# andimarafioti/qwen3-tts-cuda-graphs

Hardware: NVIDIA B200
Metric: audio_seconds_per_second (higher is better)
Workload: dtype bf16

## Files before the change

qwen3_tts_cuda_graphs_b200/csrc/fq3_api.cu:

```cuda
#include <cstdio>
#include <cstdlib>
#include <cstring>
#include <string>
#include <array>
#include <vector>

#include "../../include/fq3.h"
#include "fq3_kernel.cuh"

using namespace fq3;

namespace {

thread_local std::string g_err;
int fail(int code, const std::string& msg) {
  g_err = msg;
  return -code;
}
#define CK(call)                                                                                     \
  do {                                                                                               \
    cudaError_t _e = (call);                                                                         \
    if (_e != cudaSuccess)                                                                           \
      return fail(FQ3_E_CUDA, std::string(#call) + ": " + cudaGetErrorString(_e) + " @" + __FILE__ + ":" + \
                                  std::to_string(__LINE__));                                         \
// ... 198 lines not shown
        p.in_buf = BUF_PIN; p.out_buf = BUF_PX; p.w_off = off16(e->desc.s2m_w_off); p.b_off = off16(e->desc.s2m_b_off);
        p.N = e->pr.d.hidden; p.K = e->tk.d.hidden;
        p.plan = plan_id(e, p.N, p.K, false);
        v.push_back(p);
      }
      for (int l = 0; l < L; ++l) push_layer(e, v, e->pr, ST_PRED, l, false, (uint8_t)i, true);
    }
    Phase h{};
    h.type = PH_GEMV; h.stack = ST_PRED; h.aux = (uint8_t)i;
    h.flags = F_PRENORM | F_OUT_F32 | F_L2_KEEP;
    h.in_buf = BUF_PX; h.out_buf = BUF_LOGITS; h.w_off = off16(e->lm_head_offs[i]);
    h.g_off = off16(e->pr.d.final_norm_off); h.N = e->pr.d.vocab; h.K = e->pr.d.hidden;
    h.plan = plan_id(e, h.N, h.K, false);
    v.push_back(h);
    Phase sm{};
    sm.type = PH_SAMPLE; sm.stack = ST_PRED; sm.aux = (uint8_t)i; sm.skind = SMP_PRED;
    v.push_back(sm);
  }
}

void push_talker(std::vector<Phase>& v, fq3_engine* e, bool last_row_head) {
  for (int l = 0; l < e->tk.d.n_layers; ++l) push_layer(e, v, e->tk, ST_TALKER, l, false, 0, false);
  Phase h{};
  h.type = PH_GEMV; h.stack = ST_TALKER;
  h.flags = F_PRENORM | F_OUT_F32 | F_WRITE_NORMED | (last_row_head ? F_LAST_ROW : 0);
  h.in_buf = BUF_TX; h.out_buf = BUF_LOGITS; h.w_off = off16(e->desc.codec_head_off);
  h.g_off = off16(e->tk.d.final_norm_off); h.N = e->tk.d.vocab; h.K = e->tk.d.hidden;
  h.plan = plan_id(e, h.N, h.K, false);
  v.push_back(h);
}

int upload(fq3_engine* e, std::vector<Phase>& v, Phase** d) {
  const uint8_t* arena = reinterpret_cast<const uint8_t*>(e->desc.arena);
  std::vector<std::array<uint32_t, 8>> kinds;
  for (Phase& ph : v) {
    if (ph.type != PH_GEMV) continue;
    const std::array<uint32_t, 8> key{ph.flags, ph.in_buf, ph.out_buf, ph.res_buf, ph.N, ph.K, ph.plan, ph.b_off};
    size_t k = 0;
    while (k < kinds.size() && kinds[k] != key) ++k;
    if (k == kinds.size()) kinds.push_back(key);
    if (k >= (size_t)kMaxKinds) return -1;
    ph.kind = (uint8_t)k;
  }
  for (Phase& ph : v) {
    if (ph.type != PH_GEMV) continue;
    if (ph.N % 8) return -1;
    const uint64_t aoff = (uint64_t)ph.w_off * 16;
    uint64_t ioff = ~0ull;
    for (auto& m : e->tiled_map)
      if (m.first == aoff) ioff = m.second;
    if (ioff == ~0ull) {
      size_t used = 0;
      if (!e->tiled_map.empty()) used = e->tiled_used;
      ioff = used;
      const size_t bytes = (size_t)ph.N * ph.K * 2;
      if (ioff + bytes > e->tiled_bytes) return -1;
      fq3_tile_weights_kernel<<<256, 256>>>(reinterpret_cast<const bf16*>(arena + aoff), reinterpret_cast<uint4*>(e->tiled + ioff), (int)ph.N,
                                            (int)ph.K);
      if (cudaGetLastError() != cudaSuccess) return -1;
      e->tiled_map.push_back({aoff, ioff});
      e->tiled_used = (ioff + bytes + 1023) / 1024 * 1024;
    }
    ph.w_off = off16(ioff);
  }
  if (dalloc(e, d, v.size(), false)) return -1;
  if (cudaMemcpy(*d, v.data(), v.size() * sizeof(Phase), cudaMemcpyHostToDevice) != cudaSuccess) return -1;
  return 0;
}

void fill_common(fq3_engine* e, LaunchParams& p) {
  p.arena = reinterpret_cast<const uint8_t*>(e->desc.arena);
  p.tiled = e->tiled;
  for (int i = 0; i < kNumBufs; ++i) { p.bufs[i] = e->bufs[i]; p.ld[i] = e->ld[i]; }
  p.stacks[0] = e->rt[0];
  p.stacks[1] = e->rt[1];
  p.st = e->d_st;
  p.attn_part = e->attn_part;
  for (size_t i = 0; i < e->plans.size(); ++i) p.plans[i] = e->plans[i];
  p.err = e->err_dev;
  p.n_code_groups = e->desc.n_code_groups;
  p.eos_id = e->desc.eos_id;
  p.has_s2m = e->desc.has_s2m;
  p.max_frames = e->desc.max_frames;
  p.codec_embed = reinterpret_cast<const bf16*>(p.arena + e->desc.codec_embed_off);
  for (int i = 0; i < e->ncb; ++i) p.pred_embeds[i] = reinterpret_cast<const bf16*>(p.arena + e->pred_embed_offs[i]);
  p.pred_logits_all = nullptr;
  p.pos_override = -1;
  p.watchdog_ns = e->watchdog_ns;
  p.debug = (16 << 16) | 32;
  p.prof = e->prof;
  p.prof_cta = e->prof_cta;
  if (const char* d = getenv("FQ3_DEBUG")) p.debug = atoi(d);
  p.n_iters = 1;
  p.stream0 = 0;
  p.wide = 0;
  p.max_streams = e->desc.max_streams;
}

int check_device_fault(fq3_engine* e) {
  if (e->err_host && e->err_host[0] != 0) {
    char b[256];
    snprintf(b, sizeof b, "device watchdog fault: code=%d cta=%d phase=%d detail=%d (1=grid barrier 2=ring full-wait "
                          "3=ring empty-wait 4=frame handshake 5=bad phase)",
             e->err_host[0], e->err_host[1], e->err_host[2], e->err_host[3]);
    return fail(FQ3_E_DEVICE_FAULT, b);
  }
  return 0;
}

int phase_rows_host(const Phase& ph, int n_rows) {
  if (ph.flags & F_LAST_ROW) return 1;
  return (ph.flags & F_ROWS2) ? 2 * n_rows : n_rows;
}

int reserve_epochs(fq3_engine* e, uint64_t span, cudaStream_t s) {
  if (int r = check_device_fault(e)) return r;
  if ((uint64_t)e->epoch + span >= 0xFFFFFF00ull) {
    for (int i = 0; i < kNumBufs; ++i)
      if (e->buf_bytes[i]) fq3_ll_clear_epochs_kernel<<<64, 256, 0, s>>>(reinterpret_cast<LLWord*>(e->bufs[i]), e->buf_bytes[i] / sizeof(LLWord));
    fq3_ll_clear_epochs_kernel<<<64, 256, 0, s>>>(e->attn_part, e->attn_part_bytes / sizeof(LLWord));
    fq3_ctl_clear_epochs_kernel<<<1, 64, 0, s>>>(e->d_st, e->desc.max_streams);
    e->launches += 2;
    CK(cudaGetLastError());
    e->epoch = 1;
  }
  return 0;
}

long carve(fq3_engine* e, LaunchParams& p, const Phase* prog_host) {
  size_t xbytes = 0, gamma_elems = 0;
  for (int i = 0; i < p.n_phases; ++i) {
    const Phase& ph = prog_host[i];
    if (ph.type != PH_GEMV) continue;
    const int M = phase_rows_host(ph, p.n_rows);
    if (M > (p.wide ? kMaxWide : kMaxRows)) return fail(FQ3_E_UNSUPPORTED, "more activation rows than the GEMV stage takes");
    xbytes = std::max(xbytes, (M == 1 && !p.wide) ? (size_t)4 * ph.K : (size_t)M * ((size_t)ph.K * 2 + 64));
    if (ph.flags & F_PRENORM) gamma_elems = std::max(gamma_elems, (size_t)ph.K);
  }
  p.xbuf_bytes = (int)round_up(xbytes, 2048);
  p.prog_bytes = (int)round_up((size_t)kKindBytes + kUnitBytes + (size_t)p.n_phases * sizeof(Phase), 1024);
  p.gam_bytes = (int)round_up(gamma_elems * 2, 1024);
  const long fixed = kHeaderBytes + kScratchBytes + (long)p.xbuf_bytes + (long)p.prog_bytes + (long)kGammaSlots * p.gam_bytes;
  const long budget = e->ring_cap > 0 ? (long)e->smem_max : std::min<long>((long)e->smem_max, 196L * 1024);
  long avail = budget - fixed;
  if (avail < 6L * kStageBytes) avail = (long)e->smem_max - fixed;
  if (e->ring_cap > 0) avail = std::min(avail, e->ring_cap);
  p.n_stages = (int)std::min<long>(kMaxStages, avail / kStageBytes);
  if (p.n_stages < 2) return fail(FQ3_E_INVALID, "not enough shared memory for the weight ring");
  return fixed;
}

int launch(fq3_engine* e, LaunchParams& p, const Phase* prog_host, cudaStream_t s) {
  const int grid = e->G;
  const long fixed = carve(e, p, prog_host);
  if (fixed < 0) return (int)fixed;
  p.n_kinds = 0;
  for (int i = 0; i < p.n_phases; ++i) {
    const Phase& ph = prog_host[i];
    if (ph.type != PH_GEMV) continue;
    if (ph.kind >= kMaxKinds) return fail(FQ3_E_INVALID, "phase kind out of range");
    if (ph.kind >= p.n_kinds) {
      p.n_kinds = ph.kind + 1;
      p.kind_phase[ph.kind] = (uint16_t)i;
    }
  }
  const size_t smem = (size_t)fixed + (size_t)p.n_stages * kStageBytes;
  for (int i = 0; i < p.n_phases; ++i) {
    const Phase& ph = prog_host[i];
    if (ph.type != PH_GEMV) continue;
    Plan& pl = p.plans[ph.plan];
    if (pl.spg > p.n_stages) return fail(FQ3_E_UNSUPPORTED, "K too large for the weight ring");
    const int g_max = pl.g_base + (pl.g_rem ? 1 : 0);
    const bool follow_ref = p.mode == MODE_FRAMES && (p.wide || p.n_rows > 1) && e->ref_stages > 0;
    if (follow_ref && std::min(pl.gpr, g_max) * pl.spg > e->ref_stages) {
      pl.gpr = e->ref_stages / pl.spg;
      pl.wpg = std::max(1, std::min(kConsumerWarps / pl.gpr, pl.nch));
    }
    if (std::min(pl.gpr, g_max) * pl.spg > p.n_stages) {
      pl.gpr = p.n_stages / pl.spg;
      if (!follow_ref) pl.wpg = std::max(1, std::min(kConsumerWarps / pl.gpr, pl.nch));
    }
  }

  const uint64_t span = (uint64_t)p.n_iters * (uint64_t)p.n_phases + 2;
  if ((uint64_t)e->epoch + span >= 0xFFFFFFF0ull) return fail(FQ3_E_INVALID, "LL epochs were not reserved for this launch");
  p.epoch_base = e->epoch;
  e->epoch += (uint32_t)span;
  void* args[] = {&p};
  void* fn = p.wide ? (void*)fq3_stream_kernel<false, true> : (p.prof ? (void*)fq3_stream_kernel<true, false> : (void*)fq3_stream_kernel<false, false>);
  CK(cudaLaunchCooperativeKernel(fn, dim3(grid), dim3(kThreads), args, smem, s));
  e->launches += 1;
  e->frames_rows = (p.mode == MODE_FRAMES && !p.wide) ? p.n_rows : 0;
  return 0;
}

int pack_ll(fq3_engine* e, int buf, int row0, const void* src, int ld_src, int rows, int cols, cudaStream_t s) {
  LLWord* dst = reinterpret_cast<LLWord*>(e->bufs[buf]) + (size_t)row0 * e->ld[buf];
  const int n = rows * cols;
  fq3_pack_ll_kernel<<<std::max(1, std::min(64, (n + 255) / 256)), 256, 0, s>>>(dst, e->ld[buf], reinterpret_cast<const bf16*>(src),
                                                                          ld_src, rows, cols);
  e->launches += 1;
  CK(cudaGetLastError());
  return 0;
}
int unpack_f32(fq3_engine* e, void* dst, int ld_dst, int buf, int row0, int rows, int cols, cudaStream_t s) {
  const LLWord* src = reinterpret_cast<const LLWord*>(e->bufs[buf]) + (size_t)row0 * e->ld[buf];
  const int n = rows * cols;
  fq3_unpack_ll_f32_kernel<<<std::max(1, std::min(64, (n + 255) / 256)), 256, 0, s>>>(reinterpret_cast<float*>(dst), ld_dst, src,
                                                                                e->ld[buf], rows, cols);
  e->launches += 1;
  CK(cudaGetLastError());
  return 0;
}
int unpack_bf16(fq3_engine* e, void* dst, int ld_dst, int buf, int row0, int rows, int cols, cudaStream_t s) {
  const LLWord* src = reinterpret_cast<const LLWord*>(e->bufs[buf]) + (size_t)row0 * e->ld[buf];
  const int n = rows * cols;
  fq3_unpack_ll_bf16_kernel<<<std::max(1, std::min(64, (n + 255) / 256)), 256, 0, s>>>(reinterpret_cast<bf16*>(dst), ld_dst, src,
                                                                                 e->ld[buf], rows, cols);
  e->launches += 1;
  CK(cudaGetLastError());
  return 0;
}

Policy to_policy(const fq3_policy* q) {
  Policy p{};
  p.do_sample = q->do_sample; p.top_k = q->top_k; p.top_p = q->top_p; p.temperature = q->temperature;
  p.rep_pen = q->repetition_penalty; p.min_new_tokens = q->min_new_tokens; p.suppress_tail = q->suppress_tail;
  p.seed = q->seed;
  return p;
}
SubPolicy to_sub(const fq3_subpolicy* q) {
  SubPolicy p{};
  p.do_sample = q->do_sample; p.top_k = q->top_k; p.top_p = q->top_p; p.temperature = q->temperature;
  return p;
}

int sync_pin_layout(fq3_engine* e, int s0, int n, bool to_wpin, cudaStream_t s) {
  const int pb = e->desc.has_s2m ? BUF_PIN : BUF_PX;
  for (int i = s0; i < s0 + n; ++i) {
    if ((e->in_wpin[i] != 0) == to_wpin) continue;
    fq3_wpin_from_pairs_kernel<<<1, 256, 0, s>>>(reinterpret_cast<LLWord*>(e->bufs[BUF_WPIN]), e->ld[BUF_WPIN], reinterpret_cast<LLWord*>(e->bufs[pb]),
                                                 e->ld[pb], i, e->desc.max_streams, to_wpin ? 0 : 1);
    e->launches += 1;
    CK(cudaGetLastError());
    e->in_wpin[i] = to_wpin ? 1 : 0;
  }
  return 0;
}

int check_stack(const fq3_stack_desc& d, const char* name) {
  if (d.head_dim != kHeadDim) return fail(FQ3_E_UNSUPPORTED, std::string(name) + ": head_dim must be 128");
  if (d.hidden % 64 || d.inter % 64) return fail(FQ3_E_UNSUPPORTED, std::string(name) + ": dims must be multiples of 64");
  if (d.n_q_heads % d.n_kv_heads) return fail(FQ3_E_UNSUPPORTED, std::string(name) + ": nq % nkv != 0");
  if (d.n_q_heads / d.n_kv_heads > kGq) return fail(FQ3_E_UNSUPPORTED, std::string(name) + ": more than 2 q heads per kv head");
  if (d.vocab > kMaxVocab) return fail(FQ3_E_UNSUPPORTED, std::string(name) + ": vocab exceeds sampling scratch");
  if (d.vocab % 4) return fail(FQ3_E_UNSUPPORTED, std::string(name) + ": vocab must be a multiple of 4");
  return 0;
}

}

extern "C" {

int fq3_abi_version(void) { return FQ3_ABI_VERSION; }
const char* fq3_last_error(void) { return g_err.c_str(); }

static int create_impl(const fq3_model_desc* desc, fq3_engine* e);

int fq3_create(const fq3_model_desc* desc, fq3_engine** out) {
  if (!desc || !out) return fail(FQ3_E_INVALID, "null argument");
  *out = nullptr;
  fq3_engine* e = new fq3_engine();
  const int r = create_impl(desc, e);
  if (r) {
    const std::string msg = g_err;
    fq3_destroy(e);
    g_err = msg;
    return r;
  }
  *out = e;
  return 0;
}

static int create_impl(const fq3_model_desc* desc, fq3_engine* e) {
  if (desc->abi_version != FQ3_ABI_VERSION) return fail(FQ3_E_INVALID, "ABI version mismatch");
  if (int r = check_stack(desc->talker, "talker")) return r;
  if (int r = check_stack(desc->predictor, "predictor")) return r;
  if (desc->n_code_groups < 2 || desc->n_code_groups > FQ3_MAX_CODE_GROUPS) return fail(FQ3_E_INVALID, "n_code_groups");
  if (desc->max_streams < 1) return fail(FQ3_E_INVALID, "max_streams");
  if (!desc->has_s2m && desc->talker.hidden != desc->predictor.hidden)
    return fail(FQ3_E_INVALID, "talker/predictor widths differ but no small_to_mtp projection given");
  e->desc = *desc;
  CK(cudaGetDevice(&e->dev));
  int sms = 0, smem_optin = 0, coop = 0;
  CK(cudaDeviceGetAttribute(&sms, cudaDevAttrMultiProcessorCount, e->dev));
  CK(cudaDeviceGetAttribute(&smem_optin, cudaDevAttrMaxSharedMemoryPerBlockOptin, e->dev));
  CK(cudaDeviceGetAttribute(&coop, cudaDevAttrCooperativeLaunch, e->dev));
  if (!coop) return fail(FQ3_E_UNSUPPORTED, "device lacks cooperative launch");
  e->n_sms = sms;
  e->G = std::min(sms, 128);
  if (const char* g = getenv("FQ3_GRID")) e->G = std::max(1, std::min(sms, atoi(g)));
  if (const char* rk = getenv("FQ3_RING_KB")) e->ring_cap = std::max(16L, atol(rk)) * 1024L;
  if (const char* pc = getenv("FQ3_PROF")) {
    e->prof_cta = atoi(pc);
    if (dalloc(e, &e->prof, 512 * 160 * 2)) return -FQ3_E_CUDA;
  }
  if (const char* w = getenv("FQ3_WATCHDOG_MS")) e->watchdog_ns = (unsigned long long)atoll(w) * 1000000ull;
  e->smem_max = (size_t)smem_optin;
  CK(cudaFuncSetAttribute(fq3_stream_kernel<false, false>, cudaFuncAttributeMaxDynamicSharedMemorySize, smem_optin));
  CK(cudaFuncSetAttribute(fq3_stream_kernel<true, false>, cudaFuncAttributeMaxDynamicSharedMemorySize, smem_optin));
  CK(cudaFuncSetAttribute(fq3_stream_kernel<false, true>, cudaFuncAttributeMaxDynamicSharedMemorySize, smem_optin));
  int occ = 0;
  CK(cudaOccupancyMaxActiveBlocksPerMultiprocessor(&occ, fq3_stream_kernel<false, false>, kThreads, smem_optin));
  if (occ < 1) return fail(FQ3_E_UNSUPPORTED, "stream kernel does not fit on an SM");

  e->ncb = desc->n_code_groups - 1;
  e->tk.d = desc->talker;
  e->pr.d = desc->predictor;
  e->tk.offs.assign(desc->talker.layer_offs, desc->talker.layer_offs + (size_t)desc->talker.n_layers * 8);
  e->pr.offs.assign(desc->predictor.layer_offs, desc->predictor.layer_offs + (size_t)desc->predictor.n_layers * 8);
  e->lm_head_offs.assign(desc->lm_head_offs, desc->lm_head_offs + e->ncb);
  e->pred_embed_offs.assign(desc->pred_embed_offs, desc->pred_embed_offs + e->ncb);
  e->tk.d.layer_offs = nullptr;
  e->pr.d.layer_offs = nullptr;

  const int B = desc->max_streams;
  const int R = std::max(2 * B, 2 * kMaxRows);
  e->max_rows = R;
  const uint8_t* arena = reinterpret_cast<const uint8_t*>(desc->arena);
  for (int s = 0; s < 2; ++s) {
    const StackHost& sh = s == 0 ? e->tk : e->pr;
    StackRt& r = e->rt[s];
    r.hidden = sh.d.hidden; r.inter = sh.d.inter; r.n_layers = sh.d.n_layers; r.nq = sh.d.n_q_heads;
    r.nkv = sh.d.n_kv_heads; r.vocab = sh.d.vocab; r.eps = sh.d.rms_eps; r.max_pos = sh.d.max_pos;
    r.rope_len = sh.d.rope_len; r.n_slots = B;
    const size_t n = (size_t)sh.d.n_layers * B * sh.d.n_kv_heads * sh.d.max_pos * kHeadDim;
    if (dalloc(e, &r.kcache, n)) return -FQ3_E_CUDA;
    if (dalloc(e, &r.vcache, n)) return -FQ3_E_CUDA;
    r.rope_cos = reinterpret_cast<const bf16*>(arena + sh.d.rope_cos_off);
    r.rope_sin = reinterpret_cast<const bf16*>(arena + sh.d.rope_sin_off);
  }
  auto mk = [&](int id, int width, size_t elt, int rows) -> int {
    void* q = nullptr;
    if (dalloc(e, reinterpret_cast<uint8_t**>(&q), (size_t)rows * width * elt)) return -1;
    e->bufs[id] = q;
    e->ld[id] = width;
    e->buf_bytes[id] = (size_t)rows * width * elt;
    return 0;
  };
  const int Ht = e->tk.d.hidden, Hp = e->pr.d.hidden;
  const size_t LL = sizeof(LLWord);
  if (mk(BUF_TX, Ht / 2, LL, R) || mk(BUF_TQKV, e->tk.qkvdim() / 2, LL, R) || mk(BUF_TATT, e->tk.qdim() / 2, LL, R) ||
      mk(BUF_TACT, e->tk.d.inter / 2, LL, R) || mk(BUF_PX, Hp / 2, LL, R) || mk(BUF_PQKV, e->pr.qkvdim() / 2, LL, R) ||
      mk(BUF_PATT, e->pr.qdim() / 2, LL, R) || mk(BUF_PACT, e->pr.d.inter / 2, LL, R) ||
      mk(BUF_LOGITS, std::max(e->tk.d.vocab, e->pr.d.vocab) / 2, LL, R) || mk(BUF_HID, Ht, 2, R))
    return -FQ3_E_CUDA;
  e->buf_bytes[BUF_HID] = 0;
  if (desc->has_s2m) {
    if (mk(BUF_PIN, Ht / 2, LL, R)) return -FQ3_E_CUDA;
  } else {
    e->bufs[BUF_PIN] = e->bufs[BUF_PX];
    e->ld[BUF_PIN] = e->ld[BUF_PX];
  }
  if (mk(BUF_WPIN, Ht / 2, LL, 2 * B)) return -FQ3_E_CUDA;
  e->lin_words = 32768;
  if (mk(BUF_LIN_IN, e->lin_words, LL, kMaxRows) || mk(BUF_LIN_OUT, e->lin_words, LL, kMaxRows) ||
      mk(BUF_LIN_RES, e->lin_words, LL, kMaxRows))
    return -FQ3_E_CUDA;
  const int nqmax = std::max(e->tk.d.n_q_heads, e->pr.d.n_q_heads);
  e->attn_part_bytes = (size_t)R * nqmax * kMaxSplits * kPartStride * sizeof(LLWord);
  if (dalloc(e, &e->attn_part, (size_t)R * nqmax * kMaxSplits * kPartStride)) return -FQ3_E_CUDA;
  if (dalloc(e, &e->pred_logits_all, (size_t)e->ncb * e->pr.d.vocab)) return -FQ3_E_CUDA;
  if (dalloc(e, &e->seen_scratch, (size_t)kMaxVocab * 4)) return -FQ3_E_CUDA;
  CK(cudaHostAlloc(reinterpret_cast<void**>(&e->err_host), 64, cudaHostAllocMapped));
  memset(e->err_host, 0, 64);
  CK(cudaHostGetDevicePointer(reinterpret_cast<void**>(&e->err_dev), e->err_host, 0));
  e->h_st.resize(B);
  e->in_wpin.assign(B, 0);
  e->spol_on.assign(B, 0);
  e->text_rows.assign(B, 0);
  e->text_open.assign(B, 0);
  if (dalloc(e, &e->d_st, B)) return -FQ3_E_CUDA;
  if (dalloc(e, &e->d_spol, B)) return -FQ3_E_CUDA;
  for (int b = 0; b < B; ++b) {
    StreamState& s = e->h_st[b];
    memset(&s, 0, sizeof s);
    bf16 *tr = nullptr, *pe = nullptr;
    if (dalloc(e, &tr, (size_t)e->tk.d.max_pos * Ht)) return -FQ3_E_CUDA;
    if (dalloc(e, &pe, (size_t)Ht)) return -FQ3_E_CUDA;
    if (dalloc(e, &s.held, (size_t)Ht)) return -FQ3_E_CUDA;
    if (dalloc(e, &s.codes, (size_t)desc->max_frames * desc->n_code_groups)) return -FQ3_E_CUDA;
    if (dalloc(e, &s.seen, (size_t)round_up(e->tk.d.vocab, 16))) return -FQ3_E_CUDA;
    s.trailing = tr;
    s.pad_embed = pe;
  }
  CK(cudaMemcpy(e->d_st, e->h_st.data(), sizeof(StreamState) * B, cudaMemcpyHostToDevice));
  auto gemv_bytes = [&](const StackHost& sh) {
    return (size_t)sh.d.n_layers * ((size_t)sh.qkvdim() * sh.d.hidden + (size_t)sh.d.hidden * sh.qdim() + 3ull * sh.d.hidden * sh.d.inter) * 2;
  };
  e->tiled_bytes = gemv_bytes(e->tk) + gemv_bytes(e->pr) + (size_t)e->tk.d.vocab * e->tk.d.hidden * 2 +
                   (size_t)e->ncb * e->pr.d.vocab * e->pr.d.hidden * 2 + (desc->has_s2m ? (size_t)e->pr.d.hidden * e->tk.d.hidden * 2 : 0) +
                   1024 * (size_t)(8 * (e->tk.d.n_layers + e->pr.d.n_layers) + e->ncb + 8);
  if (dalloc(e, &e->tiled, e->tiled_bytes, false)) return -FQ3_E_CUDA;
  std::vector<Phase>& v = e->h_frames;
  push_predictor(v, e, false);
  push_talker(v, e, false);
  {
    Phase s{};
    s.type = PH_SAMPLE; s.stack = ST_TALKER; s.skind = SMP_TALKER;
    v.push_back(s);
  }
  push_predictor(e->h_pred, e, true);
  push_talker(e->h_talker, e, false);
  push_talker(e->h_prefill, e, true);
  {
    Phase s{};
    s.type = PH_SAMPLE; s.stack = ST_TALKER; s.skind = SMP_PREFILL;
    e->h_prefill.push_back(s);
  }
  push_predictor_wide(e->h_wide, e);
  push_talker(e->h_wide, e, false);
  {
    Phase s{};
    s.type = PH_SAMPLE; s.stack = ST_TALKER; s.skind = SMP_TALKER;
    e->h_wide.push_back(s);
  }
  if (g_plan_fail) { g_plan_fail = false; return fail(FQ3_E_UNSUPPORTED, "a GEMV shape of this model cannot be partitioned (odd N or K % 64)"); }
  e->n_frames_ph = (int)e->h_frames.size();
  e->n_pred_ph = (int)e->h_pred.size();
  e->n_talker_ph = (int)e->h_talker.size();
  e->n_prefill_ph = (int)e->h_prefill.size();
  e->n_wide_ph = (int)e->h_wide.size();
  if (upload(e, e->h_wide, &e->d_wide)) return fail(FQ3_E_CUDA, "wide program upload");
  {
    const int kmax = std::max(e->tk.kmax(), e->pr.kmax());
    const long fixed = kHeaderBytes + kScratchBytes + (long)round_up((size_t)kKindBytes + kUnitBytes + (size_t)e->n_wide_ph * sizeof(Phase), 1024) +
                       (long)kGammaSlots * (long)round_up((size_t)std::max(e->tk.d.hidden, e->pr.d.hidden) * 2, 1024);
    const long spg_max = ((long)kmax * 16 + kStageBytes - 1) / kStageBytes;
    const long avail = (long)e->smem_max - fixed - std::max(4L, spg_max + 1) * kStageBytes - 2048;
    e->wide_rows = (int)std::max<long>(0, std::min<long>(avail / ((long)kmax * 2 + 64), kMaxWide));
  }
  {
    LaunchParams q{};
    q.n_phases = e->n_frames_ph; q.n_rows = 1;
    if (carve(e, q, e->h_frames.data()) < 0) return -FQ3_E_INVALID;
    e->ref_stages = q.n_stages;
  }
  if (upload(e, e->h_frames, &e->d_frames) || upload(e, e->h_pred, &e->d_pred) || upload(e, e->h_talker, &e->d_talker) ||
      upload(e, e->h_prefill, &e->d_prefill))
    return fail(FQ3_E_CUDA, "program upload / weight tiling (matrix rows must be a multiple of 8)");
  if (dalloc(e, &e->d_linear, 1)) return -FQ3_E_CUDA;
  CK(cudaDeviceSynchronize());
  return 0;
}

int fq3_destroy(fq3_engine* e) {
  if (!e) return 0;
  cudaDeviceSynchronize();
// ... 313 lines not shown
  if (V <= 0 || V > kMaxVocab) return fail(FQ3_E_UNSUPPORTED, "vocab exceeds sampling scratch");
  SampleArgs a{};
  a.V = V; a.do_sample = policy->do_sample; a.top_k = policy->top_k; a.top_p = policy->top_p;
  a.temperature = policy->temperature; a.rep_pen = policy->repetition_penalty; a.seen = nullptr;
  a.suppress_start = policy->suppress_tail > 0 ? std::max(0, V - policy->suppress_tail) : V;
  a.eos = eos_id; a.suppress_eos = suppress_eos; a.round_bf16 = flags & 1; a.seed = policy->seed; a.draw = draw_index;
  a.next_emb = nullptr; a.emb_row_bytes = 0;
  fq3_sample_kernel<<<1, kConsumerThreads, 0, (cudaStream_t)stream>>>(
      reinterpret_cast<const float*>(logits_f32), a, reinterpret_cast<const long long*>(history_i64), n_history,
      e->seen_scratch, reinterpret_cast<long long*>(out_token_i64));
  e->launches += 1;
  CK(cudaGetLastError());
  return 0;
}

int fq3_apply_repetition_penalty(fq3_engine* e, void* logits_f32, int V, const void* history_i64, int n_history,
                                 float penalty, int flags, void* stream) {
  if (!e || !logits_f32) return fail(FQ3_E_INVALID, "bad arguments");
  if (V <= 0 || V > kMaxVocab * 4) return fail(FQ3_E_UNSUPPORTED, "vocab exceeds scratch");
  if (penalty == 1.0f || n_history <= 0 || !history_i64) return 0;
  fq3_rep_penalty_kernel<<<1, kConsumerThreads, 0, (cudaStream_t)stream>>>(
      reinterpret_cast<float*>(logits_f32), V, reinterpret_cast<const long long*>(history_i64), n_history, penalty,
      flags & 1, e->seen_scratch);
  e->launches += 1;
  CK(cudaGetLastError());
  return 0;
}

int fq3_decode_frames(fq3_engine* e, int n_streams, int n_frames, const fq3_policy* policy, const fq3_subpolicy* sub,
                      void* stream) {
  if (!e || !policy || !sub) return fail(FQ3_E_INVALID, "bad decode arguments");
  if (n_streams < 1 || n_streams > e->desc.max_streams) return fail(FQ3_E_INVALID, "n_streams out of range");
  if (n_frames <= 0) return 0;
  int wide_from = 3;
  if (const char* wf = getenv("FQ3_WIDE_FROM")) wide_from = std::max(1, atoi(wf));
  if ((n_streams >= wide_from && e->wide_rows > kMaxRows / 2) || 2 * n_streams > kMaxRows) {
    if (e->wide_rows <= kMaxRows / 2)
      return fail(FQ3_E_UNSUPPORTED, "more than four lock-step streams do not fit this model's staging buffer: decode in groups of fq3_lockstep_group()");
    const int n_groups = (n_streams + e->wide_rows - 1) / e->wide_rows;
    const int per = (n_streams + n_groups - 1) / n_groups;
    if (int r = sync_pin_layout(e, 0, n_streams, true, (cudaStream_t)stream)) return r;
    for (int s0 = 0; s0 < n_streams; s0 += per) {
      const int n = std::min(per, n_streams - s0);
      if (int r = reserve_epochs(e, (uint64_t)n_frames * (uint64_t)e->n_wide_ph + 2, (cudaStream_t)stream)) return r;
      LaunchParams p{};
      fill_common(e, p);
      p.prog = e->d_wide;
      p.n_phases = e->n_wide_ph;
      p.mode = MODE_FRAMES;
      p.wide = 1;
      p.n_rows = n;
      p.stream0 = s0;
      p.n_iters = n_frames;
      p.pol = to_policy(policy);
      p.spol = spol_for(e, s0, n);
      p.sub = to_sub(sub);
      if (int r = launch(e, p, e->h_wide.data(), (cudaStream_t)stream)) return r;
    }
    return 0;
  }
  if (int r = reserve_epochs(e, (uint64_t)n_frames * (uint64_t)e->n_frames_ph + 2, (cudaStream_t)stream)) return r;
  if (int r = sync_pin_layout(e, 0, n_streams, false, (cudaStream_t)stream)) return r;
  LaunchParams p{};
  fill_common(e, p);
  p.prog = e->d_frames;
  p.n_phases = e->n_frames_ph;
  p.mode = MODE_FRAMES;
  p.n_rows = n_streams;
  p.n_iters = n_frames;
  p.pol = to_policy(policy);
  p.spol = spol_for(e, 0, n_streams);
  p.sub = to_sub(sub);
  return launch(e, p, e->h_frames.data(), (cudaStream_t)stream);
}

int fq3_set_decode_grid(fq3_engine* e, int n_ctas) {
  if (!e) return fail(FQ3_E_INVALID, "null engine");
  if (n_ctas <= 0 || n_ctas == e->G || n_ctas == e->n_sms) return 0;
  return fail(FQ3_E_UNSUPPORTED, "the decode grid is fixed at engine creation (FQ3_GRID)");
}
int fq3_assemble_prompt(fq3_engine* e, const void* tp_rows, const void* desc_i32x4, int n_rows, const void* spk_rows,
                        const void* ref_codes_i32, void* out_bf16, void* stream) {
  if (!e || !desc_i32x4 || !out_bf16 || n_rows < 0) return fail(FQ3_E_INVALID, "bad assemble_prompt arguments");
  if (n_rows == 0) return 0;
  PromptTables tb{};
  const uint8_t* arena = reinterpret_cast<const uint8_t*>(e->desc.arena);
  tb.codec_embed = reinterpret_cast<const bf16*>(arena + e->desc.codec_embed_off);
  for (int i = 0; i < e->ncb; ++i) tb.pred_embeds[i] = reinterpret_cast<const bf16*>(arena + e->pred_embed_offs[i]);
  tb.ncb = e->ncb;
  fq3_assemble_prompt_kernel<<<n_rows, 256, 0, (cudaStream_t)stream>>>(
      reinterpret_cast<const bf16*>(tp_rows), reinterpret_cast<const int4*>(desc_i32x4), e->tk.d.hidden, tb,
      reinterpret_cast<const bf16*>(spk_rows), reinterpret_cast<const int*>(ref_codes_i32), e->desc.n_code_groups,
      reinterpret_cast<bf16*>(out_bf16));
  e->launches += 1;
  CK(cudaGetLastError());
  return 0;
}

int fq3_lockstep_group(const fq3_engine* e) { return e ? std::max(e->wide_rows, kMaxRows / 2) : 0; }
int fq3_reduced_grid(const fq3_engine* e) { return (e && e->G < e->n_sms) ? e->G : 0; }

int fq3_clear_fault(fq3_engine* e, void* stream) {
  if (!e) return fail(FQ3_E_INVALID, "null engine");
  cudaStreamSynchronize((cudaStream_t)stream);
  if (cudaGetLastError() != cudaSuccess) return fail(FQ3_E_CUDA, "the CUDA context is in an error state: rebuild the engine");
  if (e->err_host) memset(e->err_host, 0, 64);
  for (int i = 0; i < kNumBufs; ++i)
    if (e->buf_bytes[i]) CK(cudaMemsetAsync(e->bufs[i], 0, e->buf_bytes[i], (cudaStream_t)stream));
  CK(cudaMemsetAsync(e->attn_part, 0, e->attn_part_bytes, (cudaStream_t)stream));
  e->epoch = 1;
  return 0;
}

int fq3_debug_set_epoch(fq3_engine* e, uint32_t epoch) {
  if (!e || epoch == 0) return fail(FQ3_E_INVALID, "bad arguments");
  e->epoch = epoch;
  return 0;
}

int fq3_debug_read_talker_logits(fq3_engine* e, int idx, void* out_f32, void* stream) {
  if (int r = check_stream(e, idx)) return r;
  if (!out_f32) return fail(FQ3_E_INVALID, "null output");
  if (idx >= e->frames_rows)
    return fail(FQ3_E_INVALID, "the last launch was not a reference-shaped fq3_decode_frames launch that ran this stream");
  return unpack_f32(e, out_f32, e->tk.d.vocab, BUF_LOGITS, idx, 1, e->tk.d.vocab, (cudaStream_t)stream);
}

int fq3_get_status(fq3_engine* e, int idx, fq3_status* out, void* stream) {
  if (int r = check_stream(e, idx)) return r;
  cudaError_t se = cudaStreamSynchronize((cudaStream_t)stream);
  if (int r = check_device_fault(e)) return r;
  if (se != cudaSuccess) return fail(FQ3_E_CUDA, std::string("stream sync: ") + cudaGetErrorString(se));
  StreamState s;
  CK(cudaMemcpy(&s, e->d_st + idx, sizeof s, cudaMemcpyDeviceToHost));
  out->n_frames = s.n_frames; out->done = s.done; out->position = s.position; out->gen_step = s.gen_step;
  out->token = s.token; out->error = e->err_host[0];
  return 0;
}

int fq3_read_codes(fq3_engine* e, int idx, int first, int n, int32_t* codes_out, void* stream) {
  if (int r = check_stream(e, idx)) return r;
  if (first < 0 || n < 0 || first + n > e->desc.max_frames) return fail(FQ3_E_INVALID, "frame range");
  if (n == 0) return 0;
  const int g = e->desc.n_code_groups;
  CK(cudaMemcpyAsync(codes_out, e->h_st[idx].codes + (size_t)first * g, (size_t)n * g * 4, cudaMemcpyDeviceToHost,
                     (cudaStream_t)stream));
  CK(cudaStreamSynchronize((cudaStream_t)stream));
  return 0;
}

int fq3_debug_read_prof(fq3_engine* e, long long* out, int n_words) {
  if (!e || !e->prof) return fail(FQ3_E_INVALID, "profiling not enabled (FQ3_PROF)");
  CK(cudaDeviceSynchronize());
  CK(cudaMemcpy(out, e->prof, sizeof(long long) * std::min(n_words, 512 * 160 * 2), cudaMemcpyDeviceToHost));
  CK(cudaMemset(e->prof, 0, sizeof(long long) * 512 * 160 * 2));
  return 0;
}

int fq3_last_hidden(fq3_engine* e, int row, void* out_bf16, void* stream) {
  if (!e || !out_bf16 || row < 0 || row >= e->max_rows) return fail(FQ3_E_INVALID, "bad arguments");
  const int Ht = e->tk.d.hidden;
  CK(cudaMemcpyAsync(out_bf16, reinterpret_cast<const bf16*>(e->bufs[BUF_HID]) + (size_t)row * e->ld[BUF_HID], (size_t)Ht * 2,
                     cudaMemcpyDeviceToDevice, (cudaStream_t)stream));
  return 0;
}

void* fq3_codes_device_ptr(fq3_engine* e, int idx) {
  if (!e || idx < 0 || idx >= e->desc.max_streams) return nullptr;
  return e->h_st[idx].codes;
}

int fq3_linear(fq3_engine* e, const void* W, const void* x, void* y, int M, int N, int K, int flags, const void* gamma,
               float eps, const void* bias, const void* residual, void* stream) {
  if (!e || !W || !x || !y) return fail(FQ3_E_INVALID, "null argument");
  if (M < 1 || M > kMaxRows) return fail(FQ3_E_UNSUPPORTED, "M must be in [1, 8]");
  if (K % 64 || N < 2 || (N & 1) || K / 2 > e->lin_words || N / 2 > e->lin_words)
    return fail(FQ3_E_UNSUPPORTED, "K must be a multiple of 64 and N even");
  if ((flags & 8) && (N % 4)) return fail(FQ3_E_INVALID, "SwiGLU needs N to be a multiple of 4");
  Plan lin_plan{};
  if (!make_plan(e->G, N, K, (flags & 8) != 0, &lin_plan)) return fail(FQ3_E_UNSUPPORTED, "shape cannot be partitioned");
  cudaStream_t s = (cudaStream_t)stream;
  if (int r = reserve_epochs(e, 3, s)) return r;
  const size_t img_bytes = (size_t)((N + 7) / 8 * 8) * K * 2;
  if (img_bytes > e->lin_img_bytes) {
    CK(cudaStreamSynchronize(s));
    if (e->lin_img) {
      cudaFree(e->lin_img);
      for (void*& q : e->owned) if (q == e->lin_img) q = nullptr;
      e->lin_img = nullptr;
    }
    e->lin_img_bytes = 0;
    if (dalloc(e, &e->lin_img, img_bytes, false)) return -FQ3_E_CUDA;
    e->lin_img_bytes = img_bytes;
  }
  fq3_tile_weights_kernel<<<256, 256, 0, s>>>(reinterpret_cast<const bf16*>(W), reinterpret_cast<uint4*>(e->lin_img), N, K);
  e->launches += 1;
  CK(cudaGetLastError());
  Phase ph{};
  ph.type = PH_GEMV;
  ph.flags = F_ABSPTR | ((flags & 1) ? F_PRENORM : 0) | ((flags & 2) ? F_BIAS : 0) | ((flags & 4) ? F_RESID : 0) |
             ((flags & 8) ? F_SWIGLU : 0) | ((flags & 16) ? F_OUT_F32 : 0) | ((flags & 32) ? F_SILU : 0);
  ph.in_buf = BUF_LIN_IN; ph.out_buf = BUF_LIN_OUT; ph.res_buf = BUF_LIN_RES;
  ph.N = (uint32_t)N; ph.K = (uint32_t)K;
  ph.plan = (uint8_t)(kMaxPlans - 1);
  CK(cudaMemcpyAsync(e->d_linear, &ph, sizeof ph, cudaMemcpyHostToDevice, s));
  LaunchParams p{};
  fill_common(e, p);
  p.prog = e->d_linear;
  p.n_phases = 1;
  p.mode = MODE_LINEAR;
  p.n_rows = M;
  const int No = (flags & 8) ? N / 2 : N;
  if (int r = pack_ll(e, BUF_LIN_IN, 0, x, K, M, K, s)) return r;
  if (flags & 4) {
    if (!residual) return fail(FQ3_E_INVALID, "residual flag without a residual pointer");
    if (int r = pack_ll(e, BUF_LIN_RES, 0, residual, No, M, No, s)) return r;
  }
  p.lin_W = e->lin_img; p.lin_gamma = gamma; p.lin_bias = bias; p.lin_eps = eps;
  p.plans[kMaxPlans - 1] = lin_plan;
  if (int r = launch(e, p, &ph, s)) return r;
  if (flags & 16) return unpack_f32(e, y, No, BUF_LIN_OUT, 0, M, No, s);
  return unpack_bf16(e, y, No, BUF_LIN_OUT, 0, M, No, s);
}

}
```

qwen3_tts_cuda_graphs_b200/csrc/fq3_common.cuh:

```cuda
#pragma once
#include <cuda_bf16.h>
#include <cuda_runtime.h>
#include <stdint.h>

namespace fq3 {

typedef __nv_bfloat16 bf16;

constexpr int kConsumerWarps = 12;
constexpr int kConsumerThreads = kConsumerWarps * 32;
constexpr int kThreads = kConsumerThreads + 128;
constexpr int kProducerRegs = 56;
constexpr int kConsumerRegs = 152;
constexpr int kPollWarps = 8;
constexpr int kPollThreads = kPollWarps * 32;
constexpr int kMaxStages = 16;
constexpr int kGroupRows = 8;
constexpr int kChunkK = 32;
constexpr int kBlockBytes = kGroupRows * kChunkK * 2;
constexpr int kStageBytes = 16 * 1024;
constexpr int kStageChunks = kStageBytes / kBlockBytes;
constexpr int kHeadDim = 128;
constexpr int kMaxRows = 8;
constexpr int kMaxWide = 16;
constexpr int kMaxSplits = 16;
constexpr int kSplitLen = 4 * kConsumerWarps;
constexpr int kPartStride = 132;
constexpr int kNumBufs = 16;
constexpr int kMaxVocab = 5120;
constexpr int kScratchBytes = 24 * 1024;
constexpr int kEmptyOffset = 128;
constexpr int kCtlOffset = 256;
constexpr int kFramePosIdx = 8;
constexpr int kFrameDoneIdx = 8 + kMaxWide;
constexpr int kRedOffset = 512;
constexpr int kGFullOffset = 1024;
constexpr int kGEmptyOffset = 1056;
constexpr int kStreamConstOffset = 1088;
constexpr int kHeaderBytes = 2048;
constexpr int kGammaSlots = 4;
constexpr int kMaxPlans = 24;

typedef uint2 LLWord;

enum PhaseType : uint8_t { PH_END = 0, PH_GEMV = 1, PH_ATTN = 2, PH_SAMPLE = 3 };
enum StackId : uint8_t { ST_TALKER = 0, ST_PRED = 1 };
enum SampleKind : uint8_t { SMP_PRED = 0, SMP_TALKER = 1, SMP_PREFILL = 2, SMP_PRED_ONLY = 3 };

enum PhaseFlags : uint16_t {
  F_PRENORM = 1,
  F_BIAS = 2,
  F_RESID = 4,
  F_SWIGLU = 8,
  F_OUT_F32 = 16,
  F_ROWS2 = 32,
  F_LAST_ROW = 64,
  F_WRITE_NORMED = 128,
  F_L2_KEEP = 256,
  F_ABSPTR = 512,
  F_SILU = 1024,
  F_PASS0A = 2048,
  F_WPIN_B = 4096,
  F_IN_PREV = 8192
};

struct __align__(16) Phase {
  uint8_t type;
  uint8_t stack;
  uint8_t layer;
  uint8_t aux;
  uint16_t flags;
  uint8_t in_buf, out_buf;
  uint32_t w_off;
  uint32_t g_off;
  uint32_t b_off;
  uint32_t N;
  uint32_t K;
  uint8_t res_buf;
  uint8_t skind;
  uint8_t plan;
  uint8_t kind;
};
static_assert(sizeof(Phase) == 32, "Phase must stay 32 bytes");

enum BufId : uint8_t {
  BUF_TX = 0, BUF_TQKV, BUF_TATT, BUF_TACT, BUF_PX, BUF_PQKV, BUF_PATT, BUF_PACT, BUF_PIN,
  BUF_LOGITS, BUF_HID, BUF_LIN_IN, BUF_LIN_OUT, BUF_LIN_RES, BUF_WPIN, BUF_COUNT
};

struct Plan {
  int g_base, g_rem;
  int wpg;
  int gpr;
  int spg;
  int nch;
  int ro_shift;
  float inv_k;
};
constexpr int kMaxKinds = 32;
struct __align__(16) KindDesc {
  const LLWord* in;
  int Kq, flags;
  LLWord* out;
  const LLWord* res;
  const uint32_t* bias;
  int ldout, ldres;
  int g, grp0, wpg, gpr;
  int spg, nch, ro_shift, n_stages;
  float eps, inv_k;
  int n_rounds, wpgrp;
  int M, n_words, K, fast;
  int ldin, norm, pad0, pad1;
};
static_assert(sizeof(KindDesc) == 128, "KindDesc is eight 16-byte lines");
struct __align__(16) UnitDesc {
  int wgrp, kp;
  int ch0, ch1;
};
constexpr int kKindBytes = kMaxKinds * (int)sizeof(KindDesc);
constexpr int kUnitBytes = kMaxKinds * kConsumerWarps * (int)sizeof(UnitDesc);

struct StackRt {
  int hidden, inter, n_layers, nq, nkv, vocab;
  float eps;
  int max_pos;
  int rope_len;
  int n_slots;
  bf16* kcache;
  bf16* vcache;
  const bf16* rope_cos;
  const bf16* rope_sin;
};

struct StreamState {
  int token;
  int position;
  int gen_step;
  int n_frames;
  int done;
  int n_pad;
  int rope_delta;
  int n_trailing;
  int text_open;
  unsigned long long draws;
  const bf16* trailing;
  const bf16* pad_embed;
  bf16* held;
  int* codes;
  uint8_t* seen;
  int cur_codes[32];
  LLWord ctl[4];
};

struct Policy {
  int do_sample, top_k;
  float top_p, temperature, rep_pen;
  int min_new_tokens, suppress_tail;
  unsigned long long seed;
};
struct SubPolicy {
  int do_sample, top_k;
  float top_p, temperature;
};
struct StreamPolicy {
  int on;
  Policy pol;
};

enum Mode : int { MODE_FRAMES = 0, MODE_TALKER_STEP = 1, MODE_PREDICTOR = 2, MODE_PREFILL = 3, MODE_LINEAR = 4 };

struct LaunchParams {
  const Phase* prog;
  int n_phases;
  int n_kinds;
  uint16_t kind_phase[kMaxKinds];
  int n_iters;
  int mode;
  int n_rows;
  int wide;
  int max_streams;
  int stream0;
  int pos_override;
  int pf_pos0, pf_n_pad, pf_rope_delta, pf_final;
  const uint8_t* arena;
  const uint8_t* tiled;
  void* bufs[kNumBufs];
  int ld[kNumBufs];
  StackRt stacks[2];
  StreamState* st;
  Policy pol;
  SubPolicy sub;
  const StreamPolicy* spol;
  LLWord* attn_part;
  int* err;
// ... 21 lines not shown
```

qwen3_tts_cuda_graphs_b200/csrc/fq3_kernel.cuh:

```cuda
#pragma once
#include "fq3_common.cuh"

namespace fq3 {

__device__ __forceinline__ uint32_t smem_u32(const void* p) { return (uint32_t)__cvta_generic_to_shared(p); }

__device__ __forceinline__ void mbar_init(uint64_t* bar, uint32_t count) {
  asm volatile("mbarrier.init.shared::cta.b64 [%0], %1;" ::"r"(smem_u32(bar)), "r"(count) : "memory");
}
__device__ __forceinline__ void mbar_arrive(uint64_t* bar) {
  asm volatile("mbarrier.arrive.shared::cta.b64 _, [%0];" ::"r"(smem_u32(bar)) : "memory");
}
__device__ __forceinline__ void mbar_arrive_expect_tx(uint64_t* bar, uint32_t bytes) {
  asm volatile("mbarrier.arrive.expect_tx.shared::cta.b64 _, [%0], %1;" ::"r"(smem_u32(bar)), "r"(bytes) : "memory");
}
__device__ __forceinline__ bool mbar_try_wait(uint64_t* bar, uint32_t parity) {
  uint32_t ok;
  asm volatile(
      "{\n\t.reg .pred p;\n\t"
      "mbarrier.try_wait.parity.shared::cta.b64 p, [%1], %2;\n\t"
      "selp.u32 %0, 1, 0, p;\n\t}"
      : "=r"(ok)
      : "r"(smem_u32(bar)), "r"(parity)
      : "memory");
// ... 28 lines not shown
  asm volatile("createpolicy.fractional.L2::evict_last.b64 %0, 1.0;" : "=l"(p));
  return p;
}

__device__ __forceinline__ void cbar_sync() { asm volatile("bar.sync 1, %0;" ::"n"(kConsumerThreads) : "memory"); }

__device__ __forceinline__ unsigned long long globaltimer_ns() {
  unsigned long long t;
  asm volatile("mov.u64 %0, %%globaltimer;" : "=l"(t));
  return t;
}
__device__ __forceinline__ int ld_volatile_shared_i32(const int* p) {
  int v;
  asm volatile("ld.volatile.shared.s32 %0, [%1];" : "=r"(v) : "r"(smem_u32(p)) : "memory");
  return v;
}
__device__ __forceinline__ void st_volatile_shared_i32(int* p, int v) {
  asm volatile("st.volatile.shared.s32 [%0], %1;" ::"r"(smem_u32(p)), "r"(v) : "memory");
}
__device__ __forceinline__ uint4 lds128(uint32_t addr) {
  uint4 v;
  asm volatile("ld.shared.v4.u32 {%0, %1, %2, %3}, [%4];" : "=r"(v.x), "=r"(v.y), "=r"(v.z), "=r"(v.w) : "r"(addr));
  return v;
}

__device__ __forceinline__ LLWord ll_ld(const LLWord* p) {
  LLWord w;
  asm volatile("ld.relaxed.gpu.global.v2.u32 {%0, %1}, [%2];" : "=r"(w.x), "=r"(w.y) : "l"(p) : "memory");
  return w;
}
__device__ __forceinline__ void ll_ld2(const LLWord* p, LLWord& a, LLWord& b) {
  asm volatile("ld.relaxed.gpu.global.v4.u32 {%0, %1, %2, %3}, [%4];" : "=r"(a.x), "=r"(a.y), "=r"(b.x), "=r"(b.y) : "l"(p) : "memory");
}
__device__ __forceinline__ void ll_st(LLWord* p, uint32_t payload, uint32_t ep) {
  const unsigned long long val = ((unsigned long long)ep << 32) | payload;
  asm volatile("red.relaxed.gpu.global.max.u64 [%0], %1;" ::"l"(p), "l"(val) : "memory");
}
__device__ __forceinline__ void ll_st2(LLWord* p, uint32_t pay0, uint32_t pay1, uint32_t ep) {
  ll_st(p, pay0, ep);
  ll_st(p + 1, pay1, ep);
}
__device__ __forceinline__ void ll_stf(LLWord* p, float v, uint32_t ep) { ll_st(p, __float_as_uint(v), ep); }

__device__ __forceinline__ float bf16r(float x) { return __bfloat162float(__float2bfloat16_rn(x)); }
__device__ __forceinline__ float bf_lo(uint32_t w) { return __uint_as_float(w << 16); }
__device__ __forceinline__ float bf_hi(uint32_t w) { return __uint_as_float(w & 0xffff0000u); }
__device__ __forceinline__ uint32_t pack_bf16x2(float lo, float hi) {
  __nv_bfloat162 v = __floats2bfloat162_rn(lo, hi);
  return *reinterpret_cast<uint32_t*>(&v);
}
__device__ __forceinline__ float warp_sum(float v) {
#pragma unroll
  for (int o = 16; o > 0; o >>= 1) v += __shfl_xor_sync(0xffffffffu, v, o);
  return v;
}
__device__ __forceinline__ float warp_max(float v) {
#pragma unroll
  for (int o = 16; o > 0; o >>= 1) v = fmaxf(v, __shfl_xor_sync(0xffffffffu, v, o));
  return v;
}
struct Smem {
  uint64_t* full;
  uint64_t* empty;
  int* ctl;
  float* red;
  unsigned char* scratch;
  KindDesc* kinds;
  UnitDesc* units;
  Phase* prog;
  unsigned char* gam;
  unsigned char* xbuf;
  unsigned char* ring;
};

__device__ __forceinline__ Smem carve_smem(unsigned char* base, const LaunchParams& p) {
  Smem s;
  s.full = reinterpret_cast<uint64_t*>(base);
  s.empty = reinterpret_cast<uint64_t*>(base + kEmptyOffset);
  s.ctl = reinterpret_cast<int*>(base + kCtlOffset);
  s.red = reinterpret_cast<float*>(base + kRedOffset);
  s.scratch = base + kHeaderBytes;
  s.kinds = reinterpret_cast<KindDesc*>(s.scratch + kScratchBytes);
  s.units = reinterpret_cast<UnitDesc*>(s.scratch + kScratchBytes + kKindBytes);
  s.prog = reinterpret_cast<Phase*>(s.scratch + kScratchBytes + kKindBytes + kUnitBytes);
  s.gam = s.scratch + kScratchBytes + p.prog_bytes;
  s.xbuf = s.gam + kGammaSlots * p.gam_bytes;
  s.ring = s.xbuf + p.xbuf_bytes;
  return s;
}

__device__ __noinline__ void device_fault(const LaunchParams& p, int code, int phase, int detail) {
  volatile int* e = p.err;
  if (e[0] == 0) {
    e[1] = blockIdx.x;
    e[2] = phase;
    e[3] = detail;
    e[0] = code;
  }
  __threadfence_system();
  asm volatile("trap;");
}

struct Spin {
  unsigned long long t0;
  unsigned n;
  __device__ __forceinline__ Spin() : t0(0), n(0) {}
  __device__ __forceinline__ void tick(const LaunchParams& p, int code, int phase, int detail) {
    if ((++n & 0x3ff) == 0) {
      unsigned long long t = globaltimer_ns();
      if (t0 == 0) t0 = t;
      else if (t - t0 > p.watchdog_ns) device_fault(p, code, phase, detail);
    }
  }
};

__device__ __noinline__ void mbar_wait_slow(uint64_t* bar, uint32_t parity, const LaunchParams& p, int code, int phase) {
  Spin s;
  while (!mbar_try_wait(bar, parity)) s.tick(p, code, phase, (int)parity);
}
__device__ __forceinline__ void mbar_wait(uint64_t* bar, uint32_t parity, const LaunchParams& p, int code, int phase) {
  if (mbar_try_wait(bar, parity)) return;
  mbar_wait_slow(bar, parity, p, code, phase);
}

__device__ __noinline__ LLWord ll_spin(const LLWord* ptr, uint32_t ep, const LaunchParams& p, int phase) {
  Spin s;
  LLWord w;
  unsigned tries = 0;
  do {
    if (++tries > 4) __nanosleep(40);
    s.tick(p, DE_LL_WAIT, phase, (int)ep);
    w = ll_ld(ptr);
  } while (w.y != ep);
  return w;
}
__device__ __forceinline__ uint32_t ll_check(LLWord w, const LLWord* ptr, uint32_t ep, const LaunchParams& p, int phase) {
  if (ep != 0 && w.y != ep) w = ll_spin(ptr, ep, p, phase);
  return w.x;
}
__device__ __forceinline__ uint32_t ll_wait(const LLWord* ptr, uint32_t ep, const LaunchParams& p, int phase) {
  return ll_check(ll_ld(ptr), ptr, ep, p, phase);
}

#ifndef FQ3_CHECKS
#define FQ3_CHECKS 0
#endif
#if FQ3_CHECKS
#define FQ3_ASSERT(cond, pidx, detail) do { if (!(cond)) device_fault(p, DE_ASSERT, (pidx), (detail)); } while (0)
#else
#define FQ3_ASSERT(cond, pidx, detail) do { } while (0)
#endif

__device__ __forceinline__ void prof_cta_time(const LaunchParams& p, int pidx, int k) {
  if (p.prof && p.prof_cta == -2 && threadIdx.x == 0 && pidx >= 0 && pidx < 512)
    p.prof[((size_t)pidx * 160 + blockIdx.x) * 2 + k] = (long long)globaltimer_ns();
}
__device__ __forceinline__ void prof_warp_time(const LaunchParams& p, int pidx, int k) {
  if (p.prof && p.prof_cta == -3 && blockIdx.x == 0 && (threadIdx.x & 31) == 0 && pidx >= 0 && pidx < 512)
    p.prof[((size_t)pidx * 160 + 16 * (k >> 1) + (threadIdx.x >> 5)) * 2 + (k & 1)] = clock64();
}
__device__ __forceinline__ void prof_mark(const LaunchParams& p, int pidx, int slot, int thread = 0) {
  if (p.prof && (int)threadIdx.x == thread && (int)blockIdx.x == p.prof_cta && pidx >= 0 && pidx < 512) p.prof[(size_t)pidx * 16 + slot] = clock64();
}
#ifndef FQ3_WIDE_PROF
#define FQ3_WIDE_PROF 0
#endif
__device__ __forceinline__ void prof_acc(const LaunchParams& p, int cat, long long& t, int thread = 0) {
  if (FQ3_WIDE_PROF && p.prof && (int)threadIdx.x == thread && (int)blockIdx.x == p.prof_cta) {
    const long long now = clock64();
    p.prof[cat] += now - t;
    t = now;
  }
}
constexpr int kProfLeader = (kConsumerWarps - 1) * 32;

__device__ __forceinline__ float silu_f(float x) { return __fdividef(x, 1.f + __expf(-x)); }

__device__ __forceinline__ int phase_rows(const Phase& ph, const LaunchParams& p) {
  return (ph.flags & F_ROWS2) ? 2 * p.n_rows : p.n_rows;
}

__device__ __forceinline__ uint2 ldg_keep_u2(const void* ptr, uint64_t pol) {
  uint2 v;
  asm volatile("ld.global.nc.L2::cache_hint.v2.u32 {%0, %1}, [%2], %3;" : "=r"(v.x), "=r"(v.y) : "l"(ptr), "l"(pol));
  return v;
}

__device__ __forceinline__ Phase load_phase(const Phase* prog_smem, int i) {
  union { Phase ph; uint4 q[2]; } u;
  const uint32_t a = smem_u32(prog_smem + i);
  u.q[0] = lds128(a);
  u.q[1] = lds128(a + 16u);
  return u.ph;
}

struct Ctx {
  uint32_t full, empty, red, scratch, xs, ring, gfull, gempty, gam;
  int n_stages, gam_bytes;
  uint32_t kinds, units, xhalf;
  const Phase* prog;
};
__device__ __forceinline__ Ctx make_ctx(unsigned char* smem_base, const LaunchParams& p) {
  const Smem sm = carve_smem(smem_base, p);
  Ctx c;
  c.full = smem_u32(sm.full);
  c.empty = smem_u32(sm.empty);
  c.red = smem_u32(sm.red);
  c.scratch = smem_u32(sm.scratch);
  c.xs = smem_u32(sm.xbuf);
  c.ring = smem_u32(sm.ring);
  c.n_stages = p.n_stages;
  c.gfull = smem_u32(smem_base + kGFullOffset);
  c.gempty = smem_u32(smem_base + kGEmptyOffset);
  c.gam = smem_u32(sm.gam);
  c.gam_bytes = p.gam_bytes;
  c.xhalf = (uint32_t)p.xbuf_bytes / 2u;
  c.kinds = smem_u32(sm.kinds);
  c.units = smem_u32(sm.units);
  c.prog = sm.prog;
  return c;
}
__device__ __forceinline__ bool mbar_try_wait_a(uint32_t bar, uint32_t parity) {
  uint32_t ok;
  asm volatile(
      "{\n\t.reg .pred p;\n\t"
      "mbarrier.try_wait.parity.shared::cta.b64 p, [%1], %2;\n\t"
      "selp.u32 %0, 1, 0, p;\n\t}"
      : "=r"(ok)
      : "r"(bar), "r"(parity)
      : "memory");
  return ok != 0;
}
__device__ __forceinline__ void mbar_arrive_a(uint32_t bar) { asm volatile("mbarrier.arrive.shared::cta.b64 _, [%0];" ::"r"(bar) : "memory"); }
__device__ __forceinline__ float lds_f32(uint32_t a) {
  float v;
  asm volatile("ld.shared.f32 %0, [%1];" : "=f"(v) : "r"(a));
  return v;
}
__device__ __forceinline__ float2 lds_f32x2(uint32_t a) {
  float2 v;
  asm volatile("ld.shared.v2.f32 {%0, %1}, [%2];" : "=f"(v.x), "=f"(v.y) : "r"(a));
  return v;
}
__device__ __forceinline__ float4 lds_f32x4(uint32_t a) {
  float4 v;
  asm volatile("ld.shared.v4.f32 {%0, %1, %2, %3}, [%4];" : "=f"(v.x), "=f"(v.y), "=f"(v.z), "=f"(v.w) : "r"(a));
  return v;
}
__device__ __forceinline__ void sts_f32(uint32_t a, float v) { asm volatile("st.shared.f32 [%0], %1;" ::"r"(a), "f"(v) : "memory"); }
__device__ __forceinline__ void sts_f32x2(uint32_t a, float v0, float v1) { asm volatile("st.shared.v2.f32 [%0], {%1, %2};" ::"r"(a), "f"(v0), "f"(v1) : "memory"); }
__device__ __forceinline__ void sts_u32(uint32_t a, uint32_t v) { asm volatile("st.shared.u32 [%0], %1;" ::"r"(a), "r"(v) : "memory"); }
__device__ __forceinline__ uint32_t lds_u32(uint32_t a) {
  uint32_t v;
  asm volatile("ld.shared.u32 %0, [%1];" : "=r"(v) : "r"(a));
  return v;
}
__device__ __forceinline__ uint2 lds_u32x2(uint32_t a) {
  uint2 v;
  asm volatile("ld.shared.v2.u32 {%0, %1}, [%2];" : "=r"(v.x), "=r"(v.y) : "r"(a));
  return v;
}
__device__ __forceinline__ void group_bar_sync(int id, int nthreads) { asm volatile("bar.sync %0, %1;" ::"r"(id), "r"(nthreads) : "memory"); }

__device__ __forceinline__ void mma_bf16(float (&c)[4], uint32_t a0, uint32_t a1, uint32_t a2, uint32_t a3, uint32_t b0, uint32_t b1) {
  asm volatile(
      "mma.sync.aligned.m16n8k16.row.col.f32.bf16.bf16.f32 {%0, %1, %2, %3}, {%4, %5, %6, %7}, {%8, %9}, {%0, %1, %2, %3};"
      : "+f"(c[0]), "+f"(c[1]), "+f"(c[2]), "+f"(c[3])
      : "r"(a0), "r"(a1), "r"(a2), "r"(a3), "r"(b0), "r"(b1));
}

struct RingCur {
  int slot;
  uint32_t lap;
  __device__ __forceinline__ void advance(int n, int n_stages) {
    slot += n;
    while (slot >= n_stages) { slot -= n_stages; lap ^= 1u; }
  }
};

__device__ __forceinline__ int small_div(int a, int b) { return (int)__fdividef((float)a + 0.5f, (float)b); }

struct Slab {
  int g, grp0;
  int n_stages;
};
__device__ __forceinline__ Slab get_slab(const Phase& ph, const LaunchParams& p) {
  const Plan& pl = p.plans[ph.plan];
  const int cta = blockIdx.x;
  Slab s;
  s.g = pl.g_base + (cta < pl.g_rem ? 1 : 0);
  s.grp0 = cta * pl.g_base + min(cta, pl.g_rem);
  s.n_stages = s.g * pl.spg;
  return s;
}

__device__ __forceinline__ void resolve_kind(const LaunchParams& p, const Phase& ph, KindDesc& kd) {
  const Plan& pl = p.plans[ph.plan];
  const Slab sb = get_slab(ph, p);
  const uint32_t flags = ph.flags;
  int M = (flags & F_ROWS2) ? 2 * p.n_rows : p.n_rows, row_off = 0;
  if (flags & F_LAST_ROW) { row_off = M - 1; M = 1; }
  const int K = (int)ph.K;
  const int wpin_row = p.stream0 + ((flags & F_WPIN_B) ? p.max_streams : 0);
  if (ph.in_buf == BUF_WPIN) row_off += wpin_row;
  kd.ldin = p.ld[ph.in_buf];
  kd.in = reinterpret_cast<const LLWord*>(p.bufs[ph.in_buf]) + (size_t)row_off * kd.ldin;
  kd.Kq = K >> 2;
  kd.flags = (int)flags;
  kd.out = reinterpret_cast<LLWord*>(p.bufs[ph.out_buf]);
  kd.ldout = p.ld[ph.out_buf];
  kd.ldres = (flags & F_RESID) ? p.ld[ph.res_buf] : 0;
  kd.res = (flags & F_RESID) ? reinterpret_cast<const LLWord*>(p.bufs[ph.res_buf]) + (size_t)(ph.res_buf == BUF_WPIN ? wpin_row : 0) * kd.ldres : nullptr;
  kd.bias = nullptr;
  if (flags & F_BIAS)
    kd.bias = reinterpret_cast<const uint32_t*>((flags & F_ABSPTR) ? p.lin_bias : static_cast<const void*>(p.arena + (size_t)ph.b_off * 16));
// ... 609 lines not shown
        if (g8 + 8 < M) res_pre[1] = ll_ld(kd.res + (size_t)(g8 + 8) * kd.ldres + f_word).x;
      }
      if (flags & F_BIAS) bias_pre = __ldg(kd.bias + f_word);
    }
  }
  {
    long long* tpp = (FQ3_WIDE_PROF && p.prof) ? &tp : nullptr;
    if (K <= 1024) load_x_rows_impl<6, 1, true>(p, flags, kd.in, kd.ldin, gsrc, kd.eps, K, M, ep_in, pidx, c.xs, c.red, tpp);
    else if (K <= 2048) load_x_rows_impl<3, 2, true>(p, flags, kd.in, kd.ldin, gsrc, kd.eps, K, M, ep_in, pidx, c.xs, c.red, tpp);
    else load_x_rows_impl<2, 3, true>(p, flags, kd.in, kd.ldin, gsrc, kd.eps, K, M, ep_in, pidx, c.xs, c.red, tpp);
  }
  if (norm && lane == 0) mbar_arrive_a(gemptyb);

  const int wgrp = ud.wgrp, kp = ud.kp, ch0 = ud.ch0, ch1 = ud.ch1;
  const int wpg = kd.wpg, gpr = kd.gpr, spg = kd.spg, wpgrp = kd.wpgrp;
  const bool w_act = wgrp < gpr;
  const uint32_t rstride = xrow_stride(K);
  const uint32_t xlo = c.xs + (uint32_t)min(g8, M - 1) * rstride + (uint32_t)t * 16u;
  const uint32_t xhi = c.xs + (uint32_t)min(g8 + 8, M - 1) * rstride + (uint32_t)t * 16u;
  const uint32_t lane_w = (uint32_t)lane * 16u;
  const uint32_t pdst = c.scratch + (uint32_t)((wgrp * wpg + kp) * 64 + lane) * 8u;
#pragma unroll 1
  for (int r = 0; r < kd.n_rounds; ++r) {
    if (r != 0) cbar_sync();
    const int gi = r * gpr + wgrp;
    if (!(w_act && gi < kd.g)) continue;
    RingCur my = cur;
    my.advance(gi * spg + (ch0 >> 5), c.n_stages);
    {
      const uint32_t fb = c.full + (uint32_t)my.slot * 8u;
      Spin spin;
      while (!mbar_try_wait_a(fb, my.lap)) spin.tick(p, DE_FULL_WAIT, pidx, my.slot);
    }
    uint32_t wa = c.ring + lane_w + (uint32_t)my.slot * kStageBytes + (uint32_t)(ch0 & (kStageChunks - 1)) * kBlockBytes;
    float acc[4] = {0.f, 0.f, 0.f, 0.f}, acc2[4] = {0.f, 0.f, 0.f, 0.f};
    int ch = ch0;
    long long tq = (FQ3_WIDE_PROF && p.prof) ? clock64() : 0ll;
    if (FQ3_WIDE_PROF && p.prof) { tq = tp; prof_acc(p, 8, tq, kProfLeader); }
#pragma unroll 1
    while (ch < ch1) {
      if (ch != ch0 && (ch & (kStageChunks - 1)) == 0) {
        my.advance(1, c.n_stages);
        const uint32_t fb = c.full + (uint32_t)my.slot * 8u;
        Spin spin;
        while (!mbar_try_wait_a(fb, my.lap)) spin.tick(p, DE_FULL_WAIT, pidx, my.slot);
        wa = c.ring + lane_w + (uint32_t)my.slot * kStageBytes;
      }
      const int ce = min(ch1, (ch | (kStageChunks - 1)) + 1);
      uint32_t xa = (uint32_t)ch * kXBlock;
      uint4 wv = lds128(wa), xl = lds128(xlo + xa), xh = lds128(xhi + xa);
#pragma unroll 2
      for (int n = ce - ch - 1; n > 0; --n) {
        wa += kBlockBytes;
        xa += kXBlock;
        const uint4 wn = lds128(wa), xln = lds128(xlo + xa), xhn = lds128(xhi + xa);
        mma_bf16(acc, xl.x, xh.x, xl.y, xh.y, wv.x, wv.y);
        mma_bf16(acc2, xl.z, xh.z, xl.w, xh.w, wv.z, wv.w);
        wv = wn; xl = xln; xh = xhn;
      }
      mma_bf16(acc, xl.x, xh.x, xl.y, xh.y, wv.x, wv.y);
      mma_bf16(acc2, xl.z, xh.z, xl.w, xh.w, wv.z, wv.w);
      wa += kBlockBytes;
      ch = ce;
    }
    float y[4] = {acc[0] + acc2[0], acc[1] + acc2[1], acc[2] + acc2[2], acc[3] + acc2[3]};
    prof_acc(p, 9, tq, kProfLeader);
    if (wpg > 1) {
      if (kp != 0) {
        sts_f32x2(pdst, y[0], y[1]);
        sts_f32x2(pdst + 256u, y[2], y[3]);
      }
      group_bar_sync(2 + wgrp, wpg * 32);
      if (kp == 1) {
        if (lane == 0) {
          int rs = cur.slot + gi * spg;
          while (rs >= c.n_stages) rs -= c.n_stages;
          for (int s2 = 0; s2 < spg; ++s2) {
            mbar_arrive_a(c.empty + (uint32_t)rs * 8u);
            if (++rs == c.n_stages) rs = 0;
          }
        }
      } else if (kp == 0) {
        if (wpg <= 4) {
#pragma unroll
          for (int k2 = 1; k2 < 4; ++k2) {
            if (k2 < wpg) {
              const float2 v0 = lds_f32x2(pdst + (uint32_t)k2 * 512u), v1 = lds_f32x2(pdst + (uint32_t)k2 * 512u + 256u);
              y[0] += v0.x; y[1] += v0.y; y[2] += v1.x; y[3] += v1.y;
            }
          }
        } else {
          const float2 v0 = tree_parts(y[0], y[1], pdst, 512u, wpg), v1 = tree_parts(y[2], y[3], pdst + 256u, 512u, wpg);
          y[0] = v0.x; y[1] = v0.y; y[2] = v1.x; y[3] = v1.y;
        }
      }
    }
    prof_acc(p, 10, tq, kProfLeader);
    if (kp == 0) {
      const int f_word = (kd.grp0 + gi) * wpgrp + f_sub;
#pragma unroll
      for (int h = 0; h < 2; ++h) {
        const int row = g8 + 8 * h;
        const bool f_lane = row < M && t_ok && f_word < n_words;
        const float y0 = y[2 * h], y1 = y[2 * h + 1];
        uint32_t res0 = res_pre[h], bias0 = bias_pre;
        if (f_lane && r != 0) {
          if (flags & F_RESID) res0 = ll_ld(kd.res + (size_t)row * kd.ldres + f_word).x;
          if (flags & F_BIAS) bias0 = __ldg(kd.bias + f_word);
        }
        float lo, hi;
        if (flags & F_SWIGLU) {
          const float e = bf16r(bf16r(silu_f(bf16r(y0))) * bf16r(y1));
          lo = e;
          hi = __shfl_down_sync(0xffffffffu, e, 1);
        } else {
          lo = y0; hi = y1;
          if (flags & F_BIAS) { lo += bf_lo(bias0); hi += bf_hi(bias0); }
          lo = bf16r(lo); hi = bf16r(hi);
          if (flags & F_SILU) { lo = bf16r(silu_f(lo)); hi = bf16r(silu_f(hi)); }
        }
        if (flags & F_RESID) { lo = bf16r(bf_lo(res0) + lo); hi = bf16r(bf_hi(res0) + hi); }
        if (f_lane) ll_st(kd.out + (size_t)row * kd.ldout + f_word, pack_bf16x2(lo, hi), ep);
      }
      prof_acc(p, 11, tq, kProfLeader);
      if (wpg == 1) {
        __syncwarp();
        if (lane == 0) {
          int rs = cur.slot + gi * spg;
          while (rs >= c.n_stages) rs -= c.n_stages;
          for (int s2 = 0; s2 < spg; ++s2) {
            mbar_arrive_a(c.empty + (uint32_t)rs * 8u);
            if (++rs == c.n_stages) rs = 0;
          }
        }
      }
    }
  }
  cur.advance(kd.n_stages, c.n_stages);
  gst = ((gst & 1u) ^ 1u) | 2u;
  prof_acc(p, 3, tp);
  if (FQ3_WIDE_PROF && p.prof && tid == 0 && (int)blockIdx.x == p.prof_cta) p.prof[6] += 1;
}

template <bool PROF>
__device__ __forceinline__ bool gemv_phase_produce(const Ctx& c, const Phase& ph, const LaunchParams& p, int* ctl, RingCur& cur, RingCur& gcur, uint32_t& issued,
                                                   uint32_t& gissued, int pidx, uint64_t pol_stream, uint64_t pol_keep, uint64_t pol_gamma) {
  const Slab sb = get_slab(ph, p);
  if (sb.g == 0) return true;
  const int K = (int)ph.K;
  const uint32_t gbytes = (uint32_t)K * 16u;
  const unsigned char* W = ((ph.flags & F_ABSPTR) ? reinterpret_cast<const unsigned char*>(p.lin_W) : p.tiled + (size_t)ph.w_off * 16) +
                           (size_t)sb.grp0 * gbytes;
  const uint64_t pol = (ph.flags & F_L2_KEEP) ? pol_keep : pol_stream;
  if (PROF && (int)blockIdx.x == p.prof_cta && pidx < 512) p.prof[(size_t)pidx * 16 + 4] = clock64();
  if (ph.flags & F_PRENORM) {
    const unsigned char* gp = (ph.flags & F_ABSPTR) ? reinterpret_cast<const unsigned char*>(p.lin_gamma) : p.arena + (size_t)ph.g_off * 16;
    const uint32_t gfullb = c.gfull + (uint32_t)gcur.slot * 8u, gemptyb = c.gempty + (uint32_t)gcur.slot * 8u;
    Spin spin;
    while (!mbar_try_wait_a(gemptyb, gcur.lap ^ 1u)) {
      if (ld_volatile_shared_i32(ctl) < 0) return false;
      __nanosleep(100);
      spin.tick(p, DE_EMPTY_WAIT, pidx, 100 + gcur.slot);
    }
    if (ld_volatile_shared_i32(ctl) < 0) return false;
    asm volatile("mbarrier.arrive.expect_tx.shared::cta.b64 _, [%0], %1;" ::"r"(gfullb), "r"((uint32_t)K * 2u) : "memory");
    bulk_g2s_a(c.gam + (uint32_t)gcur.slot * (uint32_t)c.gam_bytes, gp, (uint32_t)K * 2u, gfullb, pol_gamma);
    gcur.advance(1, kGammaSlots);
    ++gissued;
  }
#pragma unroll 1
  for (int gi = 0; gi < sb.g; ++gi) {
#pragma unroll 1
    for (uint32_t off = 0; off < gbytes; off += kStageBytes) {
      const uint32_t bytes = min((uint32_t)kStageBytes, gbytes - off);
      const uint32_t fullb = c.full + (uint32_t)cur.slot * 8u, emptyb = c.empty + (uint32_t)cur.slot * 8u;
      Spin spin;
      while (!mbar_try_wait_a(emptyb, cur.lap ^ 1u)) {
        if (ld_volatile_shared_i32(ctl) < 0) return false;
        __nanosleep(100);
        spin.tick(p, DE_EMPTY_WAIT, pidx, cur.slot);
      }
      if (ld_volatile_shared_i32(ctl) < 0) return false;
      asm volatile("mbarrier.arrive.expect_tx.shared::cta.b64 _, [%0], %1;" ::"r"(fullb), "r"(bytes) : "memory");
      bulk_g2s_a(c.ring + (uint32_t)cur.slot * kStageBytes, W + (size_t)gi * gbytes + off, bytes, fullb, pol);
      cur.advance(1, c.n_stages);
      ++issued;
    }
  }
  if (PROF && (int)blockIdx.x == p.prof_cta && pidx < 512) p.prof[(size_t)pidx * 16 + 5] = clock64();
  return true;
}

struct Group {
  int first_row, nrows, slot, pos0, n_pad, rope_delta;
};
__device__ __forceinline__ int num_groups(const LaunchParams& p) { return p.mode == MODE_PREFILL ? 1 : p.n_rows; }
__device__ __forceinline__ Group get_group(const Phase& ph, const LaunchParams& p, int g, const int* frame_pos) {
  Group r;
  if (p.mode == MODE_PREFILL) {
    r.first_row = 0; r.nrows = p.n_rows; r.slot = p.stream0; r.pos0 = p.pf_pos0; r.n_pad = p.pf_n_pad;
    r.rope_delta = p.pf_rope_delta;
    return r;
  }
  r.nrows = (ph.flags & F_ROWS2) ? 2 : 1;
  r.first_row = g * r.nrows;
  r.slot = p.stream0 + g;
  if (ph.stack == ST_TALKER) {
    r.pos0 = min((p.pos_override >= 0) ? p.pos_override : frame_pos[g], p.stacks[ST_TALKER].max_pos - 1);
    const int* sconst = frame_pos + (kStreamConstOffset - kCtlOffset) / 4 - kFramePosIdx;
    r.n_pad = sconst[g];
    r.rope_delta = sconst[kMaxWide + g];
  } else {
    r.pos0 = (ph.flags & (F_ROWS2 | F_PASS0A)) ? 0 : (int)ph.aux + 1;
    r.n_pad = 0;
    r.rope_delta = 0;
  }
  return r;
}
__device__ __forceinline__ int num_splits(int L, int cap) {
  const int want = (L + kSplitLen - 1) / kSplitLen;
  return max(1, min(want, cap));
}

struct RopeRegs {
  uint2 g2, c2, s2;
};
__device__ __forceinline__ RopeRegs rope_load(const bf16* gamma, const bf16* cosp, const bf16* sinp, int lane) {
  RopeRegs r;
  const uint64_t keep = policy_evict_last();
  r.g2 = ldg_keep_u2(gamma + lane * 4, keep);
  r.c2 = ldg_keep_u2(cosp + lane * 4, keep);
  r.s2 = ldg_keep_u2(sinp + lane * 4, keep);
  return r;
}
__device__ __forceinline__ void head_norm_rope(float (&x)[4], const RopeRegs& rr, float eps, int lane) {
  const uint2 g2 = rr.g2, c2 = rr.c2, s2 = rr.s2;
  float ss = x[0] * x[0] + x[1] * x[1] + x[2] * x[2] + x[3] * x[3];
  ss = warp_sum(ss);
  const float rs = rsqrtf(ss * (1.f / kHeadDim) + eps);
  const float g[4] = {bf_lo(g2.x), bf_hi(g2.x), bf_lo(g2.y), bf_hi(g2.y)};
  const float c[4] = {bf_lo(c2.x), bf_hi(c2.x), bf_lo(c2.y), bf_hi(c2.y)};
  const float sn[4] = {bf_lo(s2.x), bf_hi(s2.x), bf_lo(s2.y), bf_hi(s2.y)};
  float y[4];
#pragma unroll
  for (int i = 0; i < 4; ++i) y[i] = bf16r(bf16r(x[i] * rs) * g[i]);
#pragma unroll
  for (int i = 0; i < 4; ++i) {
    const float partner = __shfl_xor_sync(0xffffffffu, y[i], 16);
    const float rot = (lane < 16) ? -partner : partner;
    x[i] = bf16r(bf16r(y[i] * c[i]) + bf16r(rot * sn[i]));
  }
}

__device__ __forceinline__ void ll_head_wait(const LLWord* src, uint32_t ep, LLWord& a, LLWord& b, const LaunchParams& p, int phase) {
  ll_ld2(src, a, b);
  if (ep == 0) return;
  Spin spin;
  unsigned tries = 0;
  while (__any_sync(0xffffffffu, a.y != ep || b.y != ep)) {
    if (++tries > 4) __nanosleep(40);
    spin.tick(p, DE_LL_WAIT, phase, (int)ep);
    ll_ld2(src, a, b);
  }
}

constexpr int kGq = 2;
constexpr int kAttnPre = 2;
constexpr int kAttnShort = 2 * kAttnPre * kConsumerWarps;

template <bool PROF>
__device__ __forceinline__ void attn_row(const Phase& ph, const LaunchParams& p, unsigned char* smem_base, const Group& gr, int r, int kvh, int sp,
                                      int nsplit, uint32_t ep, int pidx) {
  const Smem sm = carve_smem(smem_base, p);
  const StackRt& S = p.stacks[ph.stack];
  const int warp = threadIdx.x >> 5, lane = threadIdx.x & 31;
  const int gq = S.nq / S.nkv;
  const int qb = ph.stack == ST_TALKER ? BUF_TQKV : BUF_PQKV, ab = ph.stack == ST_TALKER ? BUF_TATT : BUF_PATT;
  const LLWord* qkv = reinterpret_cast<const LLWord*>(p.bufs[qb]) + (size_t)gr.first_row * p.ld[qb];
  const int ldq = p.ld[qb];
  constexpr int HW = kHeadDim / 2;
  const size_t head_base = (((size_t)ph.layer * S.n_slots + gr.slot) * S.nkv + kvh) * (size_t)S.max_pos * kHeadDim;
  bf16* Kc = S.kcache + head_base;
  bf16* Vc = S.vcache + head_base;
  const int pos = gr.pos0 + r;
  FQ3_ASSERT(pos >= 0 && pos < S.max_pos && gr.n_pad >= 0 && gq <= kGq, pidx, 200000 + pos);
  const int L = pos + 1 - gr.n_pad;
  FQ3_ASSERT(r >= 0 && r < kMaxRows && sp >= 0 && sp < nsplit && nsplit <= kMaxSplits, pidx, 210000 + sp);
  const int per = (L + nsplit - 1) / nsplit;
  const int a = gr.n_pad + sp * per;
  const int b = min(a + per, pos + 1);
  float* qs = reinterpret_cast<float*>(sm.scratch);
  uint4* fresh = reinterpret_cast<uint4*>(sm.scratch + 1024);
  float* wp = reinterpret_cast<float*>(sm.scratch + 1024 + 4096);
  const uint32_t ep_in = ep - 1;
  const int hw = lane >> 4, dl = lane & 15;
  if (PROF) prof_mark(p, pidx, 0);

  uint4 kpre[kAttnPre], vpre[kAttnPre];
#pragma unroll
  for (int u = 0; u < kAttnPre; ++u) {
    const int i = a + warp * 2 + hw + u * 2 * kConsumerWarps;
    kpre[u] = make_uint4(0u, 0u, 0u, 0u);
    vpre[u] = kpre[u];
    if (i < b && i < gr.pos0) {
      kpre[u] = __ldcg(reinterpret_cast<const uint4*>(Kc + (size_t)i * kHeadDim) + dl);
      vpre[u] = __ldcg(reinterpret_cast<const uint4*>(Vc + (size_t)i * kHeadDim) + dl);
    }
  }
  cbar_sync();
  if (threadIdx.x < kGq * kAttnShort) wp[threadIdx.x] = -INFINITY;

  for (int it = warp; it < gq + 2 * (r + 1); it += kConsumerWarps) {
    if (it < gq) {
      const int rp = min(max(pos + gr.rope_delta, 0), S.rope_len - 1);
      const LLWord* src = qkv + (size_t)r * ldq + (kvh * gq + it) * HW + lane * 2;
      const RopeRegs rr = rope_load(reinterpret_cast<const bf16*>(p.arena + (size_t)ph.g_off * 16), S.rope_cos + (size_t)rp * kHeadDim,
                                    S.rope_sin + (size_t)rp * kHeadDim, lane);
      LLWord w0, w1;
      ll_head_wait(src, ep_in, w0, w1, p, pidx);
      float x[4] = {bf_lo(w0.x), bf_hi(w0.x), bf_lo(w1.x), bf_hi(w1.x)};
      head_norm_rope(x, rr, S.eps, lane);
      const float scale = rsqrtf((float)kHeadDim);
      *reinterpret_cast<float4*>(qs + it * kHeadDim + lane * 4) = make_float4(x[0] * scale, x[1] * scale, x[2] * scale, x[3] * scale);
    } else {
      const int r2 = (it - gq) >> 1;
      const bool is_v = ((it - gq) & 1) != 0;
      const int kp = gr.pos0 + r2;
      if (kp >= a && kp < b) {
        const LLWord* row = qkv + (size_t)r2 * ldq;
        uint2* f = reinterpret_cast<uint2*>(fresh + (size_t)r2 * 32);
        if (is_v) {
          const LLWord* vsrc = row + (S.nq + S.nkv + kvh) * HW + lane * 2;
          LLWord v0, v1;
          ll_head_wait(vsrc, ep_in, v0, v1, p, pidx);
          const uint2 vv = make_uint2(v0.x, v1.x);
          *reinterpret_cast<uint2*>(Vc + (size_t)kp * kHeadDim + lane * 4) = vv;
          f[32 + lane] = vv;
        } else {
          const int rp = min(max(kp + gr.rope_delta, 0), S.rope_len - 1);
          const LLWord* ksrc = row + (S.nq + kvh) * HW + lane * 2;
          const RopeRegs rr = rope_load(reinterpret_cast<const bf16*>(p.arena + (size_t)ph.b_off * 16), S.rope_cos + (size_t)rp * kHeadDim,
                                        S.rope_sin + (size_t)rp * kHeadDim, lane);
// ... 528 lines not shown
                if (pass == 0) attn_item_multi(ph, p, smem_base, gr, it, nsplit, ep, pidx);
              }
            } else {
              const int kvh = small_div(it, nsplit), sp = it - kvh * nsplit;
              if (pass == 0) attn_row<PROF>(ph, p, smem_base, gr, r, kvh, sp, nsplit, ep, pidx);
              else if (nsplit > 1 && sp == 0) attn_combine(ph, p, gr, r, kvh, nsplit, ep, pidx);
            }
            found = true;
            break;
          }
          base += nitems;
        }
      }
    }
  }
}

__device__ __forceinline__ uint32_t f2key(float f) {
  uint32_t u = __float_as_uint(f);
  return (u & 0x80000000u) ? ~u : (u | 0x80000000u);
}
__device__ __forceinline__ float key2f(uint32_t k) {
  uint32_t u = (k & 0x80000000u) ? (k & 0x7fffffffu) : ~k;
  return __uint_as_float(u);
}
__device__ __forceinline__ uint4 philox4x32_10(uint4 c, uint2 k) {
#pragma unroll
  for (int i = 0; i < 10; ++i) {
    const uint32_t hi0 = __umulhi(0xD2511F53u, c.x), lo0 = 0xD2511F53u * c.x;
    const uint32_t hi1 = __umulhi(0xCD9E8D57u, c.z), lo1 = 0xCD9E8D57u * c.z;
    c = make_uint4(hi1 ^ c.y ^ k.x, lo1, hi0 ^ c.w ^ k.y, lo0);
    k.x += 0x9E3779B9u;
    k.y += 0xBB67AE85u;
  }
  return c;
}

struct SampleScratch {
  float* sl;
  unsigned* hist;
  float* redf;
  int* redi;
};
__device__ __forceinline__ SampleScratch sample_scratch(unsigned char* scratch) {
  SampleScratch s;
  s.sl = reinterpret_cast<float*>(scratch);
  s.hist = reinterpret_cast<unsigned*>(scratch + 20 * 1024);
  s.redf = reinterpret_cast<float*>(scratch + 21 * 1024);
  s.redi = reinterpret_cast<int*>(scratch + 21 * 1024 + 256);
  return s;
}

__device__ __noinline__ float block_sum(float v, float* red) {
  const int warp = threadIdx.x >> 5, lane = threadIdx.x & 31;
  v = warp_sum(v);
  cbar_sync();
  if (lane == 0) red[warp] = v;
  cbar_sync();
  float t = 0.f;
#pragma unroll
  for (int w = 0; w < kConsumerWarps; ++w) t += red[w];
  return t;
}
__device__ __noinline__ float block_max(float v, float* red) {
  const int warp = threadIdx.x >> 5, lane = threadIdx.x & 31;
  v = warp_max(v);
  cbar_sync();
  if (lane == 0) red[warp] = v;
  cbar_sync();
  float t = -INFINITY;
#pragma unroll
  for (int w = 0; w < kConsumerWarps; ++w) t = fmaxf(t, red[w]);
  return t;
}
__device__ __noinline__ int block_argmax(const float* sl, int V, float* redf, int* redi, float* out_val) {
  const int warp = threadIdx.x >> 5, lane = threadIdx.x & 31;
  float bv = -INFINITY;
  int bi = 0x7fffffff;
  for (int i = threadIdx.x; i < V; i += kConsumerThreads) {
    const float x = sl[i];
    if (x > bv || (x == bv && i < bi)) { bv = x; bi = i; }
  }
#pragma unroll
  for (int o = 16; o > 0; o >>= 1) {
    const float ov = __shfl_xor_sync(0xffffffffu, bv, o);
    const int oi = __shfl_xor_sync(0xffffffffu, bi, o);
    if (ov > bv || (ov == bv && oi < bi)) { bv = ov; bi = oi; }
  }
  cbar_sync();
  if (lane == 0) { redf[warp] = bv; redi[warp] = bi; }
  cbar_sync();
  bv = redf[0]; bi = redi[0];
#pragma unroll
  for (int w = 1; w < kConsumerWarps; ++w) {
    const float ov = redf[w]; const int oi = redi[w];
    if (ov > bv || (ov == bv && oi < bi)) { bv = ov; bi = oi; }
  }
  if (out_val) *out_val = bv;
  return bi == 0x7fffffff ? 0 : bi;
}

__device__ __noinline__ float kth_largest(const float* sl, int V, int k, unsigned* hist, int* redi) {
  uint32_t prefix = 0;
  int krem = k;
  const int lane = threadIdx.x & 31;
  for (int pass = 0; pass < 4; ++pass) {
    const int shift = 24 - 8 * pass;
    cbar_sync();
    if (threadIdx.x < 256) hist[threadIdx.x] = 0;
    cbar_sync();
    for (int i = threadIdx.x; i < V; i += kConsumerThreads) {
      const uint32_t key = f2key(sl[i]);
      const bool match = (pass == 0) || ((key >> (shift + 8)) == (prefix >> (shift + 8)));
      if (match) atomicAdd(&hist[(key >> shift) & 0xffu], 1u);
    }
    cbar_sync();
    if (threadIdx.x < 32) {
      unsigned s = 0;
#pragma unroll
      for (int t = 0; t < 8; ++t) s += hist[255 - 8 * lane - t];
      unsigned incl = s;
#pragma unroll
      for (int o = 1; o < 32; o <<= 1) {
        const unsigned n = __shfl_up_sync(0xffffffffu, incl, o);
        if (lane >= o) incl += n;
      }
      const unsigned ballot = __ballot_sync(0xffffffffu, incl >= (unsigned)krem);
      const int sel = __ffs(ballot) - 1;
      if (lane == sel) {
        unsigned above = incl - s;
        int digit = 255 - 8 * lane;
        for (int t = 0; t < 8; ++t) {
          const unsigned c = hist[255 - 8 * lane - t];
          if (above + c >= (unsigned)krem) { digit = 255 - 8 * lane - t; break; }
          above += c;
        }
        redi[0] = digit;
        redi[1] = krem - (int)above;
      }
    }
    cbar_sync();
    prefix |= ((uint32_t)redi[0]) << shift;
    krem = redi[1];
  }
  cbar_sync();
  return key2f(prefix);
}

struct SampleArgs {
  int V;
  int do_sample, top_k;
  float top_p, temperature, rep_pen;
  const uint8_t* seen;
  int suppress_start;
  int eos;
  int suppress_eos;
  int round_bf16;
  unsigned long long seed, draw;
  const bf16* next_emb;
  int emb_row_bytes;
};

__device__ __noinline__ int sample_row(const float* logits_g, const LLWord* ll, uint32_t ep, const LaunchParams* lp, int pidx,
                          const SampleArgs& a, const SampleScratch& sc) {
  float* sl = sc.sl;
  const int V = a.V;
  auto prep = [&](int i, float x) {
    if (a.seen && a.rep_pen != 1.0f && __ldcg(a.seen + i)) {
      x = (x > 0.f) ? x / a.rep_pen : x * a.rep_pen;
      if (a.round_bf16) x = bf16r(x);
    }
    if (i >= a.suppress_start && i != a.eos) x = -INFINITY;
    if (a.suppress_eos && i == a.eos) x = -INFINITY;
    if (a.do_sample) {
      x = x / a.temperature;
      if (a.round_bf16) x = bf16r(x);
    }
    sl[i] = x + 0.0f;
  };
  if (ll) {
    constexpr int kLw = (kMaxVocab / 2 + kConsumerThreads - 1) / kConsumerThreads;
    const int Vw = V >> 1;
    LLWord lw[kLw];
    Spin spin;
    unsigned tries = 0;
    bool bad;
    do {
      bad = false;
#pragma unroll
      for (int j = 0; j < kLw; ++j) {
        const int wi = threadIdx.x + j * kConsumerThreads;
        if (wi < Vw) {
          lw[j] = ll_ld(ll + wi);
          bad |= (lw[j].y != ep);
        }
      }
      if (ep == 0) break;
      if (bad) {
        if (++tries > 4) __nanosleep(40);
        spin.tick(*lp, DE_LL_WAIT, pidx, (int)ep);
      }
    } while (bad);
#pragma unroll
    for (int j = 0; j < kLw; ++j) {
      const int wi = threadIdx.x + j * kConsumerThreads;
      if (wi < Vw) {
        prep(2 * wi, bf_lo(lw[j].x));
        prep(2 * wi + 1, bf_hi(lw[j].x));
      }
    }
  } else {
    for (int i = threadIdx.x; i < V; i += kConsumerThreads) prep(i, __ldcg(logits_g + i));
  }
  cbar_sync();
  float vmax;
  const int imax = block_argmax(sl, V, sc.redf, sc.redi, &vmax);
  if (!a.do_sample) return imax;
  if (a.top_k > 0 && a.top_k < V) {
    const float thr = kth_largest(sl, V, a.top_k, sc.hist, sc.redi);
    for (int i = threadIdx.x; i < V; i += kConsumerThreads)
      if (sl[i] < thr) sl[i] = -INFINITY;
    cbar_sync();
  }
  if (a.top_p < 1.0f) {
    float loc = 0.f;
    for (int i = threadIdx.x; i < V; i += kConsumerThreads) loc += expf(sl[i] - vmax);
    const float total = block_sum(loc, sc.redf);
    const bool bf = a.round_bf16;
    auto mass = [&](float x) {
      const float e = expf(x - vmax);
      return bf ? bf16r(e / total) : e;
    };
    float P = a.top_p * total;
    bool strict = false;
    if (bf) {
      const uint32_t b = __float_as_uint(bf16r(a.top_p));
      P = 0.5f * (__uint_as_float(b) + __uint_as_float(b + 0x10000u));
      strict = (b & 0x10000u) != 0;
    }
    uint32_t lo = 0u, hi = 0xffffffffu;
    for (int it = 0; it < 32; ++it) {
      const uint32_t mid = lo + ((hi - lo) >> 1);
      float msum = 0.f;
      for (int i = threadIdx.x; i < V; i += kConsumerThreads) {
        const float x = sl[i];
        if (f2key(x) >= mid) msum += mass(x);
      }
      msum = block_sum(msum, sc.redf);
      if (msum < P || (!strict && msum == P)) hi = mid; else lo = mid + 1;
    }
    const uint32_t tkey = hi;
    uint32_t bk = 0;
    for (int i = threadIdx.x; i < V; i += kConsumerThreads) {
      const uint32_t k = f2key(sl[i]);
      if (k < tkey && k > bk) bk = k;
    }
    const float bval = block_max(key2f(bk), sc.redf);
    float above = 0.f;
    for (int i = threadIdx.x; i < V; i += kConsumerThreads)
      if (f2key(sl[i]) >= tkey) above += mass(sl[i]);
    above = block_sum(above, sc.redf);
    int keep_ties = 0;
    if (bval > -INFINITY) {
      const float pe = mass(bval);
      keep_ties = (int)floorf((P - above) / pe);
      if (strict && above + (float)keep_ties * pe >= P) --keep_ties;
      if (keep_ties < 0) keep_ties = 0;
    }
    const int seg = (V + kConsumerThreads - 1) / kConsumerThreads;
    const int i0 = threadIdx.x * seg, i1 = min(V, i0 + seg);
    int cnt = 0;
    for (int i = i0; i < i1; ++i) cnt += (sl[i] == bval) ? 1 : 0;
    const int warp = threadIdx.x >> 5, lane = threadIdx.x & 31;
    int incl = cnt;
#pragma unroll
    for (int o = 1; o < 32; o <<= 1) {
      const int n = __shfl_up_sync(0xffffffffu, incl, o);
      if (lane >= o) incl += n;
    }
    cbar_sync();
    if (lane == 31) sc.redi[warp] = incl;
    cbar_sync();
    int base = 0;
    for (int w = 0; w < warp; ++w) base += sc.redi[w];
    int rank = base + incl - cnt;
    for (int i = i0; i < i1; ++i) {
      const float x = sl[i];
      if (f2key(x) >= tkey) continue;
      if (x == bval && bval > -INFINITY) {
        if (rank < keep_ties) { ++rank; continue; }
        ++rank;
      }
      if (i != imax) sl[i] = -INFINITY;
    }
    cbar_sync();
  }
  const int seg = (V + kConsumerThreads - 1) / kConsumerThreads;
  const int i0 = threadIdx.x * seg, i1 = min(V, i0 + seg);
  float loc = 0.f;
  for (int i = i0; i < i1; ++i) loc += expf(sl[i] - vmax);
  const int warp = threadIdx.x >> 5, lane = threadIdx.x & 31;
  float incl = loc;
#pragma unroll
  for (int o = 1; o < 32; o <<= 1) {
    const float n = __shfl_up_sync(0xffffffffu, incl, o);
    if (lane >= o) incl += n;
  }
  cbar_sync();
  if (lane == 31) sc.redf[warp] = incl;
  if (threadIdx.x == 0) sc.redi[16] = 0x7fffffff;
  cbar_sync();
  float base = 0.f, total = 0.f;
  for (int w = 0; w < kConsumerWarps; ++w) {
    if (w < warp) base += sc.redf[w];
    total += sc.redf[w];
  }
  const uint4 rnd = philox4x32_10(make_uint4((uint32_t)a.draw, (uint32_t)(a.draw >> 32), 0u, 0u),
                                  make_uint2((uint32_t)a.seed, (uint32_t)(a.seed >> 32)));
  const float u = (float)(rnd.x >> 8) * (1.0f / 16777216.0f);
  const float target = u * total;
  const float excl = base + incl - loc;
  if (loc > 0.f && target >= excl && target < excl + loc) {
    float c = excl;
    int pick = -1;
    for (int i = i0; i < i1; ++i) {
      const float e = expf(sl[i] - vmax);
      if (e > 0.f) { pick = i; c += e; if (target < c) break; }
    }
    if (pick >= 0) atomicMin(&sc.redi[16], pick);
  }
  cbar_sync();
  int tok = sc.redi[16];
  if (tok == 0x7fffffff) tok = imax;
  return tok;
}

__device__ __forceinline__ uint32_t bf16_key(float x) {
  const uint32_t b = __float_as_uint(x) >> 16;
  return (b & 0x8000u) ? (~b & 0xffffu) : (b | 0x8000u);
}
__device__ __forceinline__ float bf16_key_value(uint32_t k) {
  const uint32_t b = (k & 0x8000u) ? (k & 0x7fffu) : (~k & 0xffffu);
  return __uint_as_float(b << 16);
}
__device__ __noinline__ int sample_fast(const LLWord* ll, uint32_t ep, const LaunchParams* lp, int pidx, const SampleArgs& a, unsigned char* scratch) {
  const int tid = threadIdx.x, warp = tid >> 5, lane = tid & 31;
  const int V = a.V, nw = V >> 1;
  unsigned* hist = reinterpret_cast<unsigned*>(scratch);
  float* redf = reinterpret_cast<float*>(scratch + 2048);
  int* redi = reinterpret_cast<int*>(scratch + 2048 + 128);
  const int w0i = 4 * tid;
  const bool h0 = w0i < nw, h1 = w0i + 2 < nw;
  uint4 wa = make_uint4(0u, ep, 0u, ep), wb = wa;
  if (h0) wa = ll_ld_pair(ll + w0i);
  if (h1) wb = ll_ld_pair(ll + w0i + 2);
  if (tid < 256) { hist[tid] = 0u; hist[256 + tid] = 0u; }
  cbar_sync();
  if (ep != 0) {
    unsigned tries = 0;
    while ((wa.y != ep) | (wa.w != ep) | (wb.y != ep) | (wb.w != ep)) {
      if (++tries > 4) __nanosleep(32);
      if (tries > (unsigned)(lp->watchdog_ns >> 8)) device_fault(*lp, DE_LL_WAIT, pidx, (int)ep);
      if (h0 && ((wa.y != ep) | (wa.w != ep))) wa = ll_ld_pair(ll + w0i);
      if (h1 && ((wb.y != ep) | (wb.w != ep))) wb = ll_ld_pair(ll + w0i + 2);
    }
  }
  prof_mark(*lp, pidx, 1);
  prof_warp_time(*lp, pidx, 0);
  float x[8] = {bf_lo(wa.x), bf_hi(wa.x), bf_lo(wa.z), bf_hi(wa.z), bf_lo(wb.x), bf_hi(wb.x), bf_lo(wb.z), bf_hi(wb.z)};
  unsigned long long seen8 = 0ull;
  if (a.seen && a.rep_pen != 1.0f && 8 * tid < V) seen8 = __ldcg(reinterpret_cast<const unsigned long long*>(a.seen + 8 * tid));
  {
    const int V_ = a.V, sup0 = a.suppress_start, eos = a.eos, sup_eos = a.suppress_eos, smp = a.do_sample;
    const float temp = a.temperature, pen = a.rep_pen;
    const int i0 = 8 * tid;
    const bool plain = (seen8 == 0ull) && (i0 + 8 <= V_) && (i0 + 8 <= sup0) && !(sup_eos && eos >= i0 && eos < i0 + 8);
    const float rcp = __frcp_rn(temp);
    auto div_t = [&](float v) {
      const float q = v * rcp;
      return fmaf(fmaf(-q, temp, v), rcp, q);
    };
    if (i0 >= V_) {
#pragma unroll
      for (int j = 0; j < 8; ++j) x[j] = -INFINITY;
    } else if (plain) {
      if (smp) {
#pragma unroll
        for (int j = 0; j < 8; ++j) x[j] = bf16r(div_t(x[j]));
      }
    } else {
#pragma unroll
      for (int j = 0; j < 8; ++j) {
        const int i = i0 + j;
        float v = x[j];
        if ((seen8 >> (8 * j)) & 0xffull) v = bf16r((v > 0.f) ? v / pen : v * pen);
        if (i >= sup0 && i != eos) v = -INFINITY;
        if (sup_eos && i == eos) v = -INFINITY;
        if (smp && v > -INFINITY) v = bf16r(div_t(v));
        if (i >= V_) v = -INFINITY;
        x[j] = v;
      }
    }
  }
  const bool want_k = a.do_sample && a.top_k > 0 && a.top_k < V;
  uint32_t key[8];
#pragma unroll
  for (int j = 0; j < 8; ++j) key[j] = bf16_key(x[j]);
  if (want_k && 8 * tid < V) {
    const uint32_t d0 = key[0] >> 8;
    unsigned same = 0;
#pragma unroll
    for (int j = 0; j < 8; ++j) {
      const bool in = 8 * tid + j < V;
      if (in && (key[j] >> 8) == d0) ++same;
      else if (in) atomicAdd(&hist[key[j] >> 8], 1u);
    }
    if (same) atomicAdd(&hist[d0], same);
  }
  float bv = x[0];
  int bi = 8 * tid;
#pragma unroll
  for (int j = 1; j < 8; ++j)
    if (x[j] > bv) { bv = x[j]; bi = 8 * tid + j; }
#pragma unroll
  for (int o = 16; o > 0; o >>= 1) {
    const float ov = __shfl_xor_sync(0xffffffffu, bv, o);
    const int oi = __shfl_xor_sync(0xffffffffu, bi, o);
    if (ov > bv || (ov == bv && oi < bi)) { bv = ov; bi = oi; }
  }
  if (lane == 0) { redf[warp] = bv; redi[warp] = bi; }
  prof_warp_time(*lp, pidx, 1);
  cbar_sync();
  auto select = [&](unsigned* h, int krem, int slot) {
    if (warp == 0) {
      unsigned s = 0;
#pragma unroll
      for (int t = 0; t < 8; ++t) s += h[255 - 8 * lane - t];
      unsigned incl = s;
#pragma unroll
      for (int o = 1; o < 32; o <<= 1) {
        const unsigned n = __shfl_up_sync(0xffffffffu, incl, o);
        if (lane >= o) incl += n;
      }
      const unsigned ballot = __ballot_sync(0xffffffffu, incl >= (unsigned)krem);
      const int sel = __ffs(ballot) - 1;
      if (lane == sel) {
        unsigned above = incl - s;
        int digit = 255 - 8 * lane;
        for (int t = 0; t < 8; ++t) {
          const unsigned c = h[255 - 8 * lane - t];
          if (above + c >= (unsigned)krem) { digit = 255 - 8 * lane - t; break; }
          above += c;
        }
        redi[16 + 2 * slot] = digit;
        redi[17 + 2 * slot] = krem - (int)above;
      }
    }
  };
  if (want_k) select(hist, a.top_k, 0);
  float vmax = redf[0];
  int imax = redi[0];
#pragma unroll
  for (int w = 1; w < kConsumerWarps; ++w) {
    const float ov = redf[w];
    const int oi = redi[w];
    if (ov > vmax || (ov == vmax && oi < imax)) { vmax = ov; imax = oi; }
  }
  prof_mark(*lp, pidx, 2);
  if (!a.do_sample) return imax;
  float thr = -INFINITY;
  if (want_k) {
    cbar_sync();
    const uint32_t d1 = (uint32_t)redi[16];
    const int krem = redi[17];
#pragma unroll
    for (int j = 0; j < 8; ++j)
      if (8 * tid + j < V && (key[j] >> 8) == d1) atomicAdd(&hist[256 + (key[j] & 0xffu)], 1u);
    cbar_sync();
    select(hist + 256, krem, 1);
    cbar_sync();
    thr = bf16_key_value((d1 << 8) | (uint32_t)redi[18]);
  }
  if (a.next_emb && (a.top_k > 0 && a.top_k <= 64)) {
#pragma unroll
    for (int j = 0; j < 8; ++j)
      if (x[j] >= thr && x[j] > -INFINITY)
        asm volatile("cp.async.bulk.prefetch.L2.global [%0], %1;" ::"l"(reinterpret_cast<const unsigned char*>(a.next_emb) +
                                                                       (size_t)(8 * tid + j) * a.emb_row_bytes),
                     "r"(a.emb_row_bytes)
                     : "memory");
  }
  prof_mark(*lp, pidx, 4);
  float e[8], loc = 0.f;
#pragma unroll
  for (int j = 0; j < 8; ++j) {
    e[j] = (x[j] >= thr) ? expf(x[j] - vmax) : 0.f;
    loc += e[j];
  }
  float incl = loc;
#pragma unroll
  for (int o = 1; o < 32; o <<= 1) {
    const float n = __shfl_up_sync(0xffffffffu, incl, o);
    if (lane >= o) incl += n;
  }
  if (lane == 31) redf[16 + warp] = incl;
  if (tid == 0) redi[20] = 0x7fffffff;
  cbar_sync();
  float base = 0.f, total = 0.f;
#pragma unroll
  for (int w = 0; w < kConsumerWarps; ++w) {
    const float s = redf[16 + w];
    if (w < warp) base += s;
    total += s;
  }
  const uint4 rnd = philox4x32_10(make_uint4((uint32_t)a.draw, (uint32_t)(a.draw >> 32), 0u, 0u),
                                  make_uint2((uint32_t)a.seed, (uint32_t)(a.seed >> 32)));
  const float u = (float)(rnd.x >> 8) * (1.0f / 16777216.0f);
  const float target = u * total;
  const float excl = base + incl - loc;
  if (loc > 0.f && target >= excl && target < excl + loc) {
    float c = excl;
    int pick = -1;
#pragma unroll
    for (int j = 0; j < 8; ++j) {
      if (e[j] > 0.f && (pick < 0 || target >= c)) { pick = 8 * tid + j; }
      c += e[j];
    }
    if (pick >= 0) atomicMin(&redi[20], pick);
  }
  cbar_sync();
  int tok = redi[20];
  if (tok == 0x7fffffff) tok = imax;
  prof_mark(*lp, pidx, 5);
  return tok;
}

__device__ __forceinline__ int sample_ll(const LLWord* ll, uint32_t ep, const LaunchParams& p, int pidx, const SampleArgs& a, unsigned char* scratch) {
  if (a.top_p >= 1.0f && a.V <= 8 * kConsumerThreads && (a.V & 3) == 0) return sample_fast(ll, ep, &p, pidx, a, scratch);
  return sample_row(nullptr, ll, ep, &p, pidx, a, sample_scratch(scratch));
}

__device__ __forceinline__ void publish_row(LLWord* dst, const bf16* src, int n, uint32_t ep) {
  for (int c = threadIdx.x; c < (n >> 1); c += kConsumerThreads) ll_st(dst + c, __ldg(reinterpret_cast<const uint32_t*>(src) + c), ep);
}
__device__ __noinline__ void publish_held_row(LLWord* dst, const bf16* src, int n, uint32_t ep) {
  for (int c = threadIdx.x; c < (n >> 1); c += kConsumerThreads) ll_st(dst + c, __ldcg(reinterpret_cast<const uint32_t*>(src) + c), ep);
}
__device__ __noinline__ void hold_row(bf16* dst, const bf16* src, int n) {
  for (int c = threadIdx.x; c < (n >> 1); c += kConsumerThreads)
    __stcg(reinterpret_cast<uint32_t*>(dst) + c, __ldg(reinterpret_cast<const uint32_t*>(src) + c));
}

template <bool WIDE>
__device__ __forceinline__ void sample_phase(const Phase& ph, const LaunchParams& p, unsigned char* smem_base, uint32_t ep, int pidx,
                             const int* frame_done) {
  const Smem sm = carve_smem(smem_base, p);
  const SampleScratch sc = sample_scratch(sm.scratch);
  const int Ht = p.stacks[ST_TALKER].hidden;
  const int ncb = p.n_code_groups - 1;
  const uint32_t ep_in = ep - 1;
  if ((int)blockIdx.x >= (p.mode == MODE_PREFILL ? 1 : p.n_rows) && threadIdx.x == 0 && ph.skind != SMP_PRED && ph.skind != SMP_PRED_ONLY)
    __threadfence();
  for (int b = blockIdx.x; b < (p.mode == MODE_PREFILL ? 1 : p.n_rows); b += gridDim.x) {
    prof_mark(p, pidx, 0);
    cbar_sync();
    const int slot = p.stream0 + b;
    StreamState* st = p.st + slot;
    const int done = (p.mode == MODE_FRAMES) ? frame_done[b] : 0;
    LLWord* pin = reinterpret_cast<LLWord*>(p.bufs[p.has_s2m ? BUF_PIN : BUF_PX]);
    const int ldpin = p.ld[p.has_s2m ? BUF_PIN : BUF_PX];
    const LLWord* lgbuf = reinterpret_cast<const LLWord*>(p.bufs[BUF_LOGITS]);
    if (ph.skind == SMP_PRED || ph.skind == SMP_PRED_ONLY) {
      const int i = ph.aux;
      const int Vp = p.stacks[ST_PRED].vocab;
      const int lrow = (ph.flags & F_ROWS2) ? 2 * b + 1 : b;
      const LLWord* lg = lgbuf + (size_t)lrow * p.ld[BUF_LOGITS];
      if (p.pred_logits_all) {
        for (int v = threadIdx.x; v < (Vp >> 1); v += kConsumerThreads) {
          const uint32_t pay = ll_wait(lg + v, ep_in, p, pidx);
          p.pred_logits_all[(size_t)i * Vp + 2 * v] = bf_lo(pay);
          p.pred_logits_all[(size_t)i * Vp + 2 * v + 1] = bf_hi(pay);
        }
      }
      const bool own = p.spol != nullptr && __ldcg(&p.spol[slot].on) != 0;
      const unsigned long long seed = own ? __ldcg(&p.spol[slot].pol.seed) : p.pol.seed;
      SampleArgs a;
      a.V = Vp; a.do_sample = p.sub.do_sample; a.top_k = p.sub.top_k; a.top_p = p.sub.top_p;
      a.temperature = p.sub.temperature; a.rep_pen = 1.0f; a.seen = nullptr; a.suppress_start = Vp; a.eos = -1;
      a.suppress_eos = 0; a.round_bf16 = 1; a.seed = seed ^ (0x9E3779B97F4A7C15ull * (unsigned long long)(own ? 1 : slot + 1));
      a.draw = __ldcg(&st->draws) + (unsigned long long)(i + 1);
      a.next_emb = p.pred_embeds[i]; a.emb_row_bytes = Ht * 2;
      const int tok = sample_ll(lg, ep_in, p, pidx, a, sm.scratch);
      FQ3_ASSERT(tok >= 0 && tok < Vp, pidx, 100000 + tok);
      if (threadIdx.x == 0) st->cur_codes[i + 1] = tok;
      if (i + 1 < ncb) {
        publish_row(pin + (size_t)b * ldpin, p.pred_embeds[i] + (size_t)tok * Ht, Ht, ep);
      } else if (ph.skind == SMP_PRED) {
        const int nfr = __ldcg(&st->n_frames);
        const int c0 = __ldcg(&st->token);
        if (!done) {
          if (threadIdx.x < p.n_code_groups && nfr < p.max_frames) {
            const int code = (threadIdx.x == 0) ? c0 : (threadIdx.x == ncb ? tok : __ldcg(&st->cur_codes[threadIdx.x]));
            st->codes[(size_t)nfr * p.n_code_groups + threadIdx.x] = code;
          }
          if (threadIdx.x == 0) {
            st->n_frames = nfr + 1;
            st->seen[c0] = 1;
            st->draws = __ldcg(&st->draws) + 32ull;
          }
        }
        cbar_sync();
        const int gs = __ldcg(&st->gen_step);
        const int ntr = __ldcg(&st->n_trailing);
        const bf16* text = (gs < ntr) ? st->trailing + (size_t)gs * Ht : st->pad_embed;
        LLWord* tx = reinterpret_cast<LLWord*>(p.bufs[BUF_TX]) + (size_t)b * p.ld[BUF_TX];
        const uint32_t* ce = reinterpret_cast<const uint32_t*>(p.codec_embed + (size_t)c0 * Ht);
        const uint32_t* tx32 = reinterpret_cast<const uint32_t*>(text);
        for (int c = threadIdx.x; c < (Ht >> 1); c += kConsumerThreads) {
          uint32_t v = __ldg(ce + c);
          float s0 = bf_lo(v), s1 = bf_hi(v);
          for (int g = 0; g < ncb; ++g) {
            const int code = (g == ncb - 1) ? tok : __ldcg(&st->cur_codes[g + 1]);
            v = __ldg(reinterpret_cast<const uint32_t*>(p.pred_embeds[g] + (size_t)code * Ht) + c);
            s0 += bf_lo(v); s1 += bf_hi(v);
          }
          const uint32_t t = __ldg(tx32 + c);
          ll_st(tx + c, pack_bf16x2(bf16r(bf16r(s0) + bf_lo(t)), bf16r(bf16r(s1) + bf_hi(t))), ep);
        }
        if (threadIdx.x == 0 && !done) {
          const int pos = __ldcg(&st->position);
          if (pos >= p.stacks[ST_TALKER].max_pos - 1) st->done = 2;
        }
      }
    } else {
      const int Vt = p.stacks[ST_TALKER].vocab;
      const LLWord* lg = lgbuf + (size_t)b * p.ld[BUF_LOGITS];
      const int nfr = __ldcg(&st->n_frames);
      const int done_now = (ph.skind == SMP_PREFILL) ? 0 : __ldcg(&st->done);
      const bool own = p.spol != nullptr && __ldcg(&p.spol[slot].on) != 0;
      Policy pol;
      if (own) {
        const Policy* sp = &p.spol[slot].pol;
        pol.do_sample = __ldcg(&sp->do_sample); pol.top_k = __ldcg(&sp->top_k); pol.top_p = __ldcg(&sp->top_p);
        pol.temperature = __ldcg(&sp->temperature); pol.rep_pen = __ldcg(&sp->rep_pen);
        pol.min_new_tokens = __ldcg(&sp->min_new_tokens); pol.suppress_tail = __ldcg(&sp->suppress_tail); pol.seed = __ldcg(&sp->seed);
      } else {
        pol = p.pol;
      }
      SampleArgs a;
      a.V = Vt; a.do_sample = pol.do_sample; a.top_k = pol.top_k; a.top_p = pol.top_p;
      a.temperature = pol.temperature; a.rep_pen = pol.rep_pen;
      a.seen = (ph.skind == SMP_TALKER && nfr > 0) ? st->seen : nullptr;
      a.suppress_start = max(0, Vt - pol.suppress_tail); a.eos = p.eos_id;
      a.suppress_eos = (ph.skind == SMP_PREFILL) ? (pol.min_new_tokens > 0) : (nfr < pol.min_new_tokens);
      a.round_bf16 = 1;
      a.seed = pol.seed ^ (0x9E3779B97F4A7C15ull * (unsigned long long)(own ? 1 : slot + 1));
      a.draw = __ldcg(&st->draws);
      a.next_emb = p.codec_embed; a.emb_row_bytes = Ht * 2;
      int tok = sample_ll(lg, ep_in, p, pidx, a, sm.scratch);
      const bool live = !done_now;
      int new_done = done_now, new_pos = __ldcg(&st->position), new_gs = __ldcg(&st->gen_step);
      if (live) {
        if (ph.skind == SMP_TALKER) { new_pos += 1; new_gs += 1; }
        if (tok == p.eos_id) new_done = 1;
        else if (__ldcg(&st->text_open) && new_gs >= __ldcg(&st->n_trailing)) new_done = 4;
      } else {
        tok = __ldcg(&st->token);
      }
      cbar_sync();
      if (threadIdx.x == 0) {
        if (live) { st->token = tok; st->draws = a.draw + 1ull; st->position = new_pos; st->gen_step = new_gs; st->done = new_done; }
        ll_st(&st->ctl[0], (uint32_t)new_done, ep);
        ll_st(&st->ctl[1], (uint32_t)new_pos, ep);
      }
      const bf16* hid = reinterpret_cast<const bf16*>(p.bufs[BUF_HID]) + (size_t)b * p.ld[BUF_HID];
      LLWord* const hid_dst = WIDE ? reinterpret_cast<LLWord*>(p.bufs[BUF_WPIN]) + (size_t)slot * p.ld[BUF_WPIN]
                                   : pin + (size_t)(2 * slot) * ldpin;
      if (done_now == 4) {
        publish_held_row(hid_dst, st->held, Ht, ep);
      } else {
        if (new_done == 4) hold_row(st->held, hid, Ht);
        publish_row(hid_dst, hid, Ht, ep);
      }
      if constexpr (WIDE) {
        publish_row(reinterpret_cast<LLWord*>(p.bufs[BUF_WPIN]) + (size_t)(p.max_streams + slot) * p.ld[BUF_WPIN],
                    p.codec_embed + (size_t)tok * Ht, Ht, ep);
      } else {
        publish_row(pin + (size_t)(2 * slot + 1) * ldpin, p.codec_embed + (size_t)tok * Ht, Ht, ep);
      }
      if (threadIdx.x == 0) __threadfence();
    }
    prof_mark(p, pidx, 6);
    cbar_sync();
    prof_mark(p, pidx, 3);
  }
}

template <bool PROF, bool WIDE>
__global__ void __launch_bounds__(kThreads, 1) fq3_stream_kernel(const __grid_constant__ LaunchParams p) {
  extern __shared__ __align__(1024) unsigned char smem_raw[];
  const Smem sm = carve_smem(smem_raw, p);
  const Ctx c = make_ctx(smem_raw, p);
  const int tid = threadIdx.x;

  if (tid == 0) {
    for (int s = 0; s < kMaxStages; ++s) {
      mbar_init(&sm.full[s], 1);
      mbar_init(&sm.empty[s], 1);
    }
    for (int s = 0; s < kGammaSlots; ++s) {
      mbar_init(reinterpret_cast<uint64_t*>(smem_raw + kGFullOffset) + s, 1);
      mbar_init(reinterpret_cast<uint64_t*>(smem_raw + kGEmptyOffset) + s, kConsumerWarps);
    }
    sm.ctl[0] = 0;
    fence_barrier_init();
  }
  {
    const uint4* src = reinterpret_cast<const uint4*>(p.prog);
    uint4* dst = reinterpret_cast<uint4*>(sm.prog);
    for (int i = tid; i < p.n_phases * 2; i += kThreads) dst[i] = __ldg(src + i);
  }
  __syncthreads();
  if (tid < p.n_kinds) resolve_kind(p, sm.prog[p.kind_phase[tid]], sm.kinds[tid]);
  __syncthreads();
  for (int i = tid; i < p.n_kinds * kConsumerWarps; i += kThreads) resolve_unit(sm.kinds[i / kConsumerWarps], i % kConsumerWarps, sm.units[i]);
  __syncthreads();

#ifndef FQ3_SETMAXNREG
#define FQ3_SETMAXNREG 1
#endif
#if FQ3_SETMAXNREG
  if (tid >= kConsumerThreads) {
    asm volatile("setmaxnreg.dec.sync.aligned.u32 %0;" ::"n"(kProducerRegs));
  } else {
    asm volatile("setmaxnreg.inc.sync.aligned.u32 %0;" ::"n"(kConsumerRegs));
  }
#endif
  if (tid >= kConsumerThreads) {
    if (tid == kConsumerThreads) {
      const uint64_t pol_stream = policy_evict_first(), pol_keep = policy_keep_fraction();
      const uint64_t pol_gamma = policy_evict_last();
      RingCur cur{0, 0u}, gcur{0, 0u};
      uint32_t issued = 0, gissued = 0;
      bool ok = true;
      for (int iter = 0; iter < p.n_iters && ok; ++iter) {
        for (int i = 0; i < p.n_phases && ok; ++i) {
          const Phase ph = load_phase(sm.prog, i);
          if (ph.type == PH_GEMV) ok = gemv_phase_produce<PROF>(c, ph, p, sm.ctl, cur, gcur, issued, gissued, i, pol_stream, pol_keep, pol_gamma);
        }
      }
      const int n = (int)min(issued, (uint32_t)p.n_stages);
      RingCur d = cur;
      for (int k = 0; k < n; ++k) {
        if (d.slot == 0) { d.slot = p.n_stages - 1; d.lap ^= 1u; } else { --d.slot; }
        mbar_wait(&sm.full[d.slot], d.lap, p, DE_FULL_WAIT, -3);
      }
      const int gn = (int)min(gissued, (uint32_t)kGammaSlots);
      d = gcur;
      for (int k = 0; k < gn; ++k) {
        if (d.slot == 0) { d.slot = kGammaSlots - 1; d.lap ^= 1u; } else { --d.slot; }
        mbar_wait(reinterpret_cast<uint64_t*>(smem_raw + kGFullOffset) + d.slot, d.lap, p, DE_FULL_WAIT, -4);
      }
    }
    return;
  }

  RingCur cur{0, 0u}, gcur{0, 0u};
  uint32_t gst = 0u;
  int* frame_pos = sm.ctl + kFramePosIdx;
  int* frame_done = sm.ctl + kFrameDoneIdx;
  for (int iter = 0; iter < p.n_iters; ++iter) {
    const uint32_t ep0 = p.epoch_base + (uint32_t)iter * (uint32_t)p.n_phases;
    if (p.mode == MODE_FRAMES || p.mode == MODE_TALKER_STEP) {
      if (tid < p.n_rows) {
        const StreamState* st = p.st + p.stream0 + tid;
        int done, pos;
        if (iter == 0) {
          done = __ldcg(&st->done);
          pos = __ldcg(&st->position);
          int* sconst = reinterpret_cast<int*>(smem_raw + kStreamConstOffset);
          sconst[tid] = __ldcg(&st->n_pad);
          sconst[kMaxWide + tid] = __ldcg(&st->rope_delta);
        } else {
          done = (int)ll_wait(&st->ctl[0], ep0, p, -2);
          pos = (int)ll_wait(&st->ctl[1], ep0, p, -2);
        }
        frame_pos[tid] = pos;
        frame_done[tid] = done;
      }
      cbar_sync();
      if (p.mode == MODE_FRAMES && iter > 0) {
        int all_done = 1;
        for (int b = 0; b < p.n_rows; ++b) all_done &= (frame_done[b] != 0);
        if (all_done) {
          if (tid == 0) st_volatile_shared_i32(&sm.ctl[0], -1);
          break;
        }
      }
    }
    for (int i = 0; i < p.n_phases; ++i) {
      const Phase ph = load_phase(sm.prog, i);
      const uint32_t ep = ep0 + (uint32_t)i + 1u;
      switch (ph.type) {
        case PH_GEMV:
          if constexpr (WIDE) gemv_phase_consume_wide(c, ph, p, cur, gcur, gst, i, ep);
          else gemv_phase_consume<PROF>(c, ph, p, cur, gcur, gst, i, ep);
          break;
        case PH_ATTN:
          if constexpr (WIDE) {
            long long tp = (FQ3_WIDE_PROF && p.prof) ? clock64() : 0ll;
            attn_phase<PROF, true>(ph, p, smem_raw, ep, i, frame_pos);
            prof_acc(p, 4, tp);
          } else {
            attn_phase<PROF, false>(ph, p, smem_raw, ep, i, frame_pos);
          }
          break;
        case PH_SAMPLE:
          if constexpr (WIDE) {
            long long tp = (FQ3_WIDE_PROF && p.prof) ? clock64() : 0ll;
            sample_phase<WIDE>(ph, p, smem_raw, ep, i, frame_done);
            prof_acc(p, 5, tp);
          } else {
            sample_phase<WIDE>(ph, p, smem_raw, ep, i, frame_done);
          }
          break;
        default: if (tid == 0) device_fault(p, DE_BAD_PHASE, i, ph.type); break;
      }
    }
  }
}

__global__ void fq3_tile_weights_kernel(const bf16* __restrict__ W, uint4* __restrict__ out, int N, int K) {
  const long pieces = (long)((N + 7) / 8) * K;
  for (long idx = blockIdx.x * (long)blockDim.x + threadIdx.x; idx < pieces; idx += (long)gridDim.x * blockDim.x) {
    const long grp = idx / K;
    const int pc = (int)(idx - grp * K);
    const int ch = pc >> 5, ln = pc & 31, r8 = ln >> 2, t = ln & 3;
    const long row = grp * 8 + r8;
    uint4 v = make_uint4(0u, 0u, 0u, 0u);
    if (row < N) {
      const uint32_t* src = reinterpret_cast<const uint32_t*>(W + (size_t)row * K + ch * kChunkK) + t;
      v = make_uint4(__ldg(src), __ldg(src + 4), __ldg(src + 8), __ldg(src + 12));
    }
    out[idx] = v;
  }
}

__global__ void __launch_bounds__(kConsumerThreads, 1)
fq3_sample_kernel(const float* logits, SampleArgs a, const long long* history, int n_history, uint8_t* seen_scratch,
                  long long* out) {
  __shared__ __align__(16) unsigned char scratch[24 * 1024];
  const SampleScratch sc = sample_scratch(scratch);
  if (history && n_history > 0 && a.rep_pen != 1.0f) {
    for (int i = threadIdx.x; i < a.V; i += kConsumerThreads) seen_scratch[i] = 0;
    __syncthreads();
    for (int i = threadIdx.x; i < n_history; i += kConsumerThreads) {
      const long long t = history[i];
      if (t >= 0 && t < a.V) seen_scratch[t] = 1;
    }
    __syncthreads();
    a.seen = seen_scratch;
  } else {
    a.seen = nullptr;
  }
  const int tok = sample_row(logits, nullptr, 0u, nullptr, 0, a, sc);
  if (threadIdx.x == 0) out[0] = tok;
}

__global__ void __launch_bounds__(kConsumerThreads, 1)
fq3_rep_penalty_kernel(float* logits, int V, const long long* history, int n_history, float penalty, int round_bf16,
                       uint8_t* seen) {
  for (int i = threadIdx.x; i < V; i += kConsumerThreads) seen[i] = 0;
  __syncthreads();
  for (int i = threadIdx.x; i < n_history; i += kConsumerThreads) {
    const long long t = history[i];
    if (t >= 0 && t < V) seen[t] = 1;
  }
  __syncthreads();
  for (int i = threadIdx.x; i < V; i += kConsumerThreads) {
    if (__ldcg(seen + i)) {
      float x = logits[i];
      x = (x > 0.f) ? x / penalty : x * penalty;
      logits[i] = round_bf16 ? bf16r(x) : x;
    }
  }
}

__global__ void fq3_wpin_from_pairs_kernel(LLWord* wpin, int ldw, LLWord* pairs, int ldp, int slot, int max_streams, int reverse) {
  for (int c = threadIdx.x; c < ldw; c += blockDim.x) {
    LLWord* a0 = wpin + (size_t)slot * ldw + c;
    LLWord* a1 = wpin + (size_t)(max_streams + slot) * ldw + c;
    LLWord* b0 = pairs + (size_t)(2 * slot) * ldp + c;
    LLWord* b1 = pairs + (size_t)(2 * slot + 1) * ldp + c;
    if (reverse) { *b0 = make_uint2(a0->x, 0u); *b1 = make_uint2(a1->x, 0u); }
    else { *a0 = make_uint2(b0->x, 0u); *a1 = make_uint2(b1->x, 0u); }
  }
}

struct PromptTables {
  const bf16* codec_embed;
  const bf16* pred_embeds[32];
  int ncb;
};
__global__ void fq3_assemble_prompt_kernel(const bf16* __restrict__ tp, const int4* __restrict__ desc, int H, PromptTables tb,
                                           const bf16* __restrict__ spk, const int* __restrict__ ref_codes, int n_groups, bf16* __restrict__ out) {
  const int r = blockIdx.x;
  const int4 d = desc[r];
  const int Hw = H >> 1;
  uint32_t* o = reinterpret_cast<uint32_t*>(out + (size_t)r * H);
  const uint32_t* t = d.x >= 0 ? reinterpret_cast<const uint32_t*>(tp + (size_t)d.x * H) : nullptr;
  for (int c = threadIdx.x; c < Hw; c += blockDim.x) {
    float c0 = 0.f, c1 = 0.f;
    bool have_c = d.y != 0;
    if (d.y == 1) {
      const uint32_t v = __ldg(reinterpret_cast<const uint32_t*>(tb.codec_embed + (size_t)d.z * H) + c);
      c0 = bf_lo(v); c1 = bf_hi(v);
    } else if (d.y == 2) {
      const uint32_t v = __ldg(reinterpret_cast<const uint32_t*>(spk + (size_t)d.z * H) + c);
      c0 = bf_lo(v); c1 = bf_hi(v);
    } else if (d.y == 3) {
      const int* codes = ref_codes + (size_t)d.z * n_groups;
      uint32_t v = __ldg(reinterpret_cast<const uint32_t*>(tb.codec_embed + (size_t)codes[0] * H) + c);
      c0 = bf_lo(v); c1 = bf_hi(v);
// ... 104 lines not shown
```

Baseline: 46.34.

## Cache per-stream sampling state in shared memory across fused decode iterations

Loads each stream's sampling policy, counters, current codes and a bit-packed repetition-seen mask into a shared-memory context once at kernel start. Sampling phases then read and update that context instead of re-reading global StreamState with uncached loads every phase. The sampler also hoists argument decoding before the barrier, does top-k digit selection inside a warp with shuffles to drop barriers, issues the Philox draw earlier, and batches the predictor-embedding sum loads. It adds a check that the sampled streams fit the grid, since the cached state assumes one CTA per stream. It also raises the profiling table size, and the cached state relies on staying consistent with global memory.

```diff
diff --git a/qwen3_tts_cuda_graphs_b200/csrc/fq3_api.cu b/qwen3_tts_cuda_graphs_b200/csrc/fq3_api.cu
--- a/qwen3_tts_cuda_graphs_b200/csrc/fq3_api.cu
+++ b/qwen3_tts_cuda_graphs_b200/csrc/fq3_api.cu
@@ -374,6 +374,8 @@
 
 int launch(fq3_engine* e, LaunchParams& p, const Phase* prog_host, cudaStream_t s) {
   const int grid = e->G;
+  if ((p.mode == MODE_FRAMES || p.mode == MODE_PREDICTOR) && p.n_rows > grid)
+    return fail(FQ3_E_UNSUPPORTED, "more sampled streams than CTAs in the grid");
   const long fixed = carve(e, p, prog_host);
   if (fixed < 0) return (int)fixed;
   p.n_kinds = 0;
@@ -525,7 +527,7 @@
   if (const char* rk = getenv("FQ3_RING_KB")) e->ring_cap = std::max(16L, atol(rk)) * 1024L;
   if (const char* pc = getenv("FQ3_PROF")) {
     e->prof_cta = atoi(pc);
-    if (dalloc(e, &e->prof, 512 * 160 * 2)) return -FQ3_E_CUDA;
+    if (dalloc(e, &e->prof, kProfPhases * 160 * 2)) return -FQ3_E_CUDA;
   }
   if (const char* w = getenv("FQ3_WATCHDOG_MS")) e->watchdog_ns = (unsigned long long)atoll(w) * 1000000ull;
   e->smem_max = (size_t)smem_optin;
@@ -1145,8 +1147,8 @@
 int fq3_debug_read_prof(fq3_engine* e, long long* out, int n_words) {
   if (!e || !e->prof) return fail(FQ3_E_INVALID, "profiling not enabled (FQ3_PROF)");
   CK(cudaDeviceSynchronize());
-  CK(cudaMemcpy(out, e->prof, sizeof(long long) * std::min(n_words, 512 * 160 * 2), cudaMemcpyDeviceToHost));
-  CK(cudaMemset(e->prof, 0, sizeof(long long) * 512 * 160 * 2));
+  CK(cudaMemcpy(out, e->prof, sizeof(long long) * std::min(n_words, kProfPhases * 160 * 2), cudaMemcpyDeviceToHost));
+  CK(cudaMemset(e->prof, 0, sizeof(long long) * kProfPhases * 160 * 2));
   return 0;
 }
 
diff --git a/qwen3_tts_cuda_graphs_b200/csrc/fq3_common.cuh b/qwen3_tts_cuda_graphs_b200/csrc/fq3_common.cuh
--- a/qwen3_tts_cuda_graphs_b200/csrc/fq3_common.cuh
+++ b/qwen3_tts_cuda_graphs_b200/csrc/fq3_common.cuh
@@ -37,9 +37,12 @@
 constexpr int kGFullOffset = 1024;
 constexpr int kGEmptyOffset = 1056;
 constexpr int kStreamConstOffset = 1088;
+constexpr int kSampleArgsOffset = 1216;
+constexpr int kSampleCtxOffset = 1312;
 constexpr int kHeaderBytes = 2048;
 constexpr int kGammaSlots = 4;
 constexpr int kMaxPlans = 24;
+constexpr int kProfPhases = 1024;
 
 typedef uint2 LLWord;
 
diff --git a/qwen3_tts_cuda_graphs_b200/csrc/fq3_kernel.cuh b/qwen3_tts_cuda_graphs_b200/csrc/fq3_kernel.cuh
--- a/qwen3_tts_cuda_graphs_b200/csrc/fq3_kernel.cuh
+++ b/qwen3_tts_cuda_graphs_b200/csrc/fq3_kernel.cuh
@@ -204,15 +204,15 @@
 #endif
 
 __device__ __forceinline__ void prof_cta_time(const LaunchParams& p, int pidx, int k) {
-  if (p.prof && p.prof_cta == -2 && threadIdx.x == 0 && pidx >= 0 && pidx < 512)
+  if (p.prof && p.prof_cta == -2 && threadIdx.x == 0 && pidx >= 0 && pidx < kProfPhases)
     p.prof[((size_t)pidx * 160 + blockIdx.x) * 2 + k] = (long long)globaltimer_ns();
 }
 __device__ __forceinline__ void prof_warp_time(const LaunchParams& p, int pidx, int k) {
-  if (p.prof && p.prof_cta == -3 && blockIdx.x == 0 && (threadIdx.x & 31) == 0 && pidx >= 0 && pidx < 512)
+  if (p.prof && p.prof_cta == -3 && blockIdx.x == 0 && (threadIdx.x & 31) == 0 && pidx >= 0 && pidx < kProfPhases)
     p.prof[((size_t)pidx * 160 + 16 * (k >> 1) + (threadIdx.x >> 5)) * 2 + (k & 1)] = clock64();
 }
 __device__ __forceinline__ void prof_mark(const LaunchParams& p, int pidx, int slot, int thread = 0) {
-  if (p.prof && (int)threadIdx.x == thread && (int)blockIdx.x == p.prof_cta && pidx >= 0 && pidx < 512) p.prof[(size_t)pidx * 16 + slot] = clock64();
+  if (p.prof && (int)threadIdx.x == thread && (int)blockIdx.x == p.prof_cta && pidx >= 0 && pidx < kProfPhases) p.prof[(size_t)pidx * 16 + slot] = clock64();
 }
 #ifndef FQ3_WIDE_PROF
 #define FQ3_WIDE_PROF 0
@@ -1128,7 +1128,7 @@
   const unsigned char* W = ((ph.flags & F_ABSPTR) ? reinterpret_cast<const unsigned char*>(p.lin_W) : p.tiled + (size_t)ph.w_off * 16) +
                            (size_t)sb.grp0 * gbytes;
   const uint64_t pol = (ph.flags & F_L2_KEEP) ? pol_keep : pol_stream;
-  if (PROF && (int)blockIdx.x == p.prof_cta && pidx < 512) p.prof[(size_t)pidx * 16 + 4] = clock64();
+  if (PROF && (int)blockIdx.x == p.prof_cta && pidx < kProfPhases) p.prof[(size_t)pidx * 16 + 4] = clock64();
   if (ph.flags & F_PRENORM) {
     const unsigned char* gp = (ph.flags & F_ABSPTR) ? reinterpret_cast<const unsigned char*>(p.lin_gamma) : p.arena + (size_t)ph.g_off * 16;
     const uint32_t gfullb = c.gfull + (uint32_t)gcur.slot * 8u, gemptyb = c.gempty + (uint32_t)gcur.slot * 8u;
@@ -1163,7 +1163,7 @@
       ++issued;
     }
   }
-  if (PROF && (int)blockIdx.x == p.prof_cta && pidx < 512) p.prof[(size_t)pidx * 16 + 5] = clock64();
+  if (PROF && (int)blockIdx.x == p.prof_cta && pidx < kProfPhases) p.prof[(size_t)pidx * 16 + 5] = clock64();
   return true;
 }
 
@@ -1998,6 +1998,7 @@
   int do_sample, top_k;
   float top_p, temperature, rep_pen;
   const uint8_t* seen;
+  const uint8_t* seen8;
   int suppress_start;
   int eos;
   int suppress_eos;
@@ -2006,6 +2007,49 @@
   const bf16* next_emb;
   int emb_row_bytes;
 };
+static_assert(sizeof(SampleArgs) <= kSampleCtxOffset - kSampleArgsOffset, "SampleArgs slot of the shared-memory header");
+
+struct SampleCtx {
+  Policy pol;
+  unsigned long long key;
+  unsigned long long draws;
+  int token, position, gen_step, n_frames, done, text_open, n_trailing, pad;
+  int cur_codes[32];
+  uint8_t seen8[kConsumerThreads];
+};
+static_assert(kSampleCtxOffset + sizeof(SampleCtx) <= kHeaderBytes, "SampleCtx must fit the shared-memory header");
+
+__device__ __noinline__ void load_sample_ctx(const LaunchParams& p, SampleCtx* cx) {
+  const int t = threadIdx.x;
+  const int slot = p.stream0 + blockIdx.x;
+  const StreamState* st = p.st + slot;
+  if (t == 0) {
+    const bool own = p.spol != nullptr && __ldcg(&p.spol[slot].on) != 0;
+    Policy pol;
+    if (own) {
+      const Policy* sp = &p.spol[slot].pol;
+      pol.do_sample = __ldcg(&sp->do_sample); pol.top_k = __ldcg(&sp->top_k); pol.top_p = __ldcg(&sp->top_p);
+      pol.temperature = __ldcg(&sp->temperature); pol.rep_pen = __ldcg(&sp->rep_pen);
+      pol.min_new_tokens = __ldcg(&sp->min_new_tokens); pol.suppress_tail = __ldcg(&sp->suppress_tail); pol.seed = __ldcg(&sp->seed);
+    } else {
+      pol = p.pol;
+    }
+    cx->pol = pol;
+    cx->key = pol.seed ^ (0x9E3779B97F4A7C15ull * (unsigned long long)(own ? 1 : slot + 1));
+    cx->draws = __ldcg(&st->draws);
+    cx->token = __ldcg(&st->token); cx->position = __ldcg(&st->position); cx->gen_step = __ldcg(&st->gen_step);
+    cx->n_frames = __ldcg(&st->n_frames); cx->done = __ldcg(&st->done); cx->text_open = __ldcg(&st->text_open);
+    cx->n_trailing = __ldcg(&st->n_trailing);
+  }
+  if (t < 32) cx->cur_codes[t] = __ldcg(&st->cur_codes[t]);
+  unsigned m = 0u;
+  if (8 * t < p.stacks[ST_TALKER].vocab) {
+    const unsigned long long s = __ldcg(reinterpret_cast<const unsigned long long*>(st->seen + 8 * t));
+#pragma unroll
+    for (int j = 0; j < 8; ++j) m |= ((s >> (8 * j)) & 0xffull) ? (1u << j) : 0u;
+  }
+  cx->seen8[t] = (uint8_t)m;
+}
 
 __device__ __noinline__ int sample_row(const float* logits_g, const LLWord* ll, uint32_t ep, const LaunchParams* lp, int pidx,
                           const SampleArgs& a, const SampleScratch& sc) {
@@ -2189,9 +2233,9 @@
   const uint32_t b = (k & 0x8000u) ? (k & 0x7fffu) : (~k & 0xffffu);
   return __uint_as_float(b << 16);
 }
-__device__ __noinline__ int sample_fast(const LLWord* ll, uint32_t ep, const LaunchParams* lp, int pidx, const SampleArgs& a, unsigned char* scratch) {
+__device__ __noinline__ int sample_fast(const LLWord* ll, uint32_t ep, const LaunchParams* lp, int pidx, const SampleArgs* a, unsigned char* scratch) {
   const int tid = threadIdx.x, warp = tid >> 5, lane = tid & 31;
-  const int V = a.V, nw = V >> 1;
+  const int V = a->V, nw = V >> 1;
   unsigned* hist = reinterpret_cast<unsigned*>(scratch);
   float* redf = reinterpret_cast<float*>(scratch + 2048);
   int* redi = reinterpret_cast<int*>(scratch + 2048 + 128);
@@ -2201,6 +2245,13 @@
   if (h0) wa = ll_ld_pair(ll + w0i);
   if (h1) wb = ll_ld_pair(ll + w0i + 2);
   if (tid < 256) { hist[tid] = 0u; hist[256 + tid] = 0u; }
+  const int sup0 = a->suppress_start, eos = a->eos, sup_eos = a->suppress_eos, smp = a->do_sample, top_k = a->top_k;
+  const float temp = a->temperature, pen = a->rep_pen;
+  const unsigned seen8 = (a->seen8 && pen != 1.0f && 8 * tid < V) ? a->seen8[tid] : 0u;
+  const int i0 = 8 * tid;
+  const bool plain = (seen8 == 0u) && (i0 + 8 <= V) && (i0 + 8 <= sup0) && !(sup_eos && eos >= i0 && eos < i0 + 8);
+  const bool want_k = smp && top_k > 0 && top_k < V;
+  const float rcp = __frcp_rn(temp);
   cbar_sync();
   if (ep != 0) {
     unsigned tries = 0;
@@ -2214,19 +2265,12 @@
   prof_mark(*lp, pidx, 1);
   prof_warp_time(*lp, pidx, 0);
   float x[8] = {bf_lo(wa.x), bf_hi(wa.x), bf_lo(wa.z), bf_hi(wa.z), bf_lo(wb.x), bf_hi(wb.x), bf_lo(wb.z), bf_hi(wb.z)};
-  unsigned long long seen8 = 0ull;
-  if (a.seen && a.rep_pen != 1.0f && 8 * tid < V) seen8 = __ldcg(reinterpret_cast<const unsigned long long*>(a.seen + 8 * tid));
   {
-    const int V_ = a.V, sup0 = a.suppress_start, eos = a.eos, sup_eos = a.suppress_eos, smp = a.do_sample;
-    const float temp = a.temperature, pen = a.rep_pen;
-    const int i0 = 8 * tid;
-    const bool plain = (seen8 == 0ull) && (i0 + 8 <= V_) && (i0 + 8 <= sup0) && !(sup_eos && eos >= i0 && eos < i0 + 8);
-    const float rcp = __frcp_rn(temp);
     auto div_t = [&](float v) {
       const float q = v * rcp;
       return fmaf(fmaf(-q, temp, v), rcp, q);
     };
-    if (i0 >= V_) {
+    if (i0 >= V) {
 #pragma unroll
       for (int j = 0; j < 8; ++j) x[j] = -INFINITY;
     } else if (plain) {
@@ -2239,16 +2283,15 @@
       for (int j = 0; j < 8; ++j) {
         const int i = i0 + j;
         float v = x[j];
-        if ((seen8 >> (8 * j)) & 0xffull) v = bf16r((v > 0.f) ? v / pen : v * pen);
+        if ((seen8 >> j) & 1u) v = bf16r((v > 0.f) ? v / pen : v * pen);
         if (i >= sup0 && i != eos) v = -INFINITY;
         if (sup_eos && i == eos) v = -INFINITY;
         if (smp && v > -INFINITY) v = bf16r(div_t(v));
-        if (i >= V_) v = -INFINITY;
+        if (i >= V) v = -INFINITY;
         x[j] = v;
       }
     }
   }
-  const bool want_k = a.do_sample && a.top_k > 0 && a.top_k < V;
   uint32_t key[8];
 #pragma unroll
   for (int j = 0; j < 8; ++j) key[j] = bf16_key(x[j]);
@@ -2277,33 +2320,33 @@
   if (lane == 0) { redf[warp] = bv; redi[warp] = bi; }
   prof_warp_time(*lp, pidx, 1);
   cbar_sync();
-  auto select = [&](unsigned* h, int krem, int slot) {
-    if (warp == 0) {
-      unsigned s = 0;
-#pragma unroll
-      for (int t = 0; t < 8; ++t) s += h[255 - 8 * lane - t];
-      unsigned incl = s;
-#pragma unroll
-      for (int o = 1; o < 32; o <<= 1) {
-        const unsigned n = __shfl_up_sync(0xffffffffu, incl, o);
-        if (lane >= o) incl += n;
-      }
-      const unsigned ballot = __ballot_sync(0xffffffffu, incl >= (unsigned)krem);
-      const int sel = __ffs(ballot) - 1;
-      if (lane == sel) {
-        unsigned above = incl - s;
-        int digit = 255 - 8 * lane;
-        for (int t = 0; t < 8; ++t) {
-          const unsigned c = h[255 - 8 * lane - t];
-          if (above + c >= (unsigned)krem) { digit = 255 - 8 * lane - t; break; }
-          above += c;
-        }
-        redi[16 + 2 * slot] = digit;
-        redi[17 + 2 * slot] = krem - (int)above;
-      }
-    }
+  auto select = [&](const unsigned* h, int krem, uint32_t& digit_out, int& krem_out) {
+    const uint4 lo = *reinterpret_cast<const uint4*>(h + 248 - 8 * lane), hi = *reinterpret_cast<const uint4*>(h + 252 - 8 * lane);
+    const unsigned c[8] = {hi.w, hi.z, hi.y, hi.x, lo.w, lo.z, lo.y, lo.x};
+    unsigned s = 0;
+#pragma unroll
+    for (int t = 0; t < 8; ++t) s += c[t];
+    unsigned incl = s;
+#pragma unroll
+    for (int o = 1; o < 32; o <<= 1) {
+      const unsigned n = __shfl_up_sync(0xffffffffu, incl, o);
+      if (lane >= o) incl += n;
+    }
+    const unsigned ballot = __ballot_sync(0xffffffffu, incl >= (unsigned)krem);
+    const int sel = __ffs(ballot) - 1;
+    unsigned above = incl - s;
+    int digit = 255 - 8 * lane;
+    bool found = false;
+#pragma unroll
+    for (int t = 0; t < 8; ++t) {
+      if (!found) {
+        if (above + c[t] >= (unsigned)krem) { digit = 255 - 8 * lane - t; found = true; }
+        else above += c[t];
+      }
+    }
+    digit_out = (uint32_t)__shfl_sync(0xffffffffu, digit, sel);
+    krem_out = __shfl_sync(0xffffffffu, krem - (int)above, sel);
   };
-  if (want_k) select(hist, a.top_k, 0);
   float vmax = redf[0];
   int imax = redi[0];
 #pragma unroll
@@ -2313,30 +2356,29 @@
     if (ov > vmax || (ov == vmax && oi < imax)) { vmax = ov; imax = oi; }
   }
   prof_mark(*lp, pidx, 2);
-  if (!a.do_sample) return imax;
+  if (!smp) return imax;
   float thr = -INFINITY;
   if (want_k) {
-    cbar_sync();
-    const uint32_t d1 = (uint32_t)redi[16];
-    const int krem = redi[17];
+    uint32_t d1, d2;
+    int krem, krem2;
+    select(hist, top_k, d1, krem);
 #pragma unroll
     for (int j = 0; j < 8; ++j)
       if (8 * tid + j < V && (key[j] >> 8) == d1) atomicAdd(&hist[256 + (key[j] & 0xffu)], 1u);
     cbar_sync();
-    select(hist + 256, krem, 1);
-    cbar_sync();
-    thr = bf16_key_value((d1 << 8) | (uint32_t)redi[18]);
-  }
-  if (a.next_emb && (a.top_k > 0 && a.top_k <= 64)) {
+    select(hist + 256, krem, d2, krem2);
+    thr = bf16_key_value((d1 << 8) | d2);
+  }
+  const unsigned char* next_emb = reinterpret_cast<const unsigned char*>(a->next_emb);
+  if (next_emb && (top_k > 0 && top_k <= 64)) {
+    const int rb = a->emb_row_bytes;
 #pragma unroll
     for (int j = 0; j < 8; ++j)
       if (x[j] >= thr && x[j] > -INFINITY)
-        asm volatile("cp.async.bulk.prefetch.L2.global [%0], %1;" ::"l"(reinterpret_cast<const unsigned char*>(a.next_emb) +
-                                                                       (size_t)(8 * tid + j) * a.emb_row_bytes),
-                     "r"(a.emb_row_bytes)
-                     : "memory");
+        asm volatile("cp.async.bulk.prefetch.L2.global [%0], %1;" ::"l"(next_emb + (size_t)(8 * tid + j) * rb), "r"(rb) : "memory");
   }
   prof_mark(*lp, pidx, 4);
+  const unsigned long long seed = a->seed, draw = a->draw;
   float e[8], loc = 0.f;
 #pragma unroll
   for (int j = 0; j < 8; ++j) {
@@ -2351,6 +2393,7 @@
   }
   if (lane == 31) redf[16 + warp] = incl;
   if (tid == 0) redi[20] = 0x7fffffff;
+  const uint4 rnd = philox4x32_10(make_uint4((uint32_t)draw, (uint32_t)(draw >> 32), 0u, 0u), make_uint2((uint32_t)seed, (uint32_t)(seed >> 32)));
   cbar_sync();
   float base = 0.f, total = 0.f;
 #pragma unroll
@@ -2359,8 +2402,6 @@
     if (w < warp) base += s;
     total += s;
   }
-  const uint4 rnd = philox4x32_10(make_uint4((uint32_t)a.draw, (uint32_t)(a.draw >> 32), 0u, 0u),
-                                  make_uint2((uint32_t)a.seed, (uint32_t)(a.seed >> 32)));
   const float u = (float)(rnd.x >> 8) * (1.0f / 16777216.0f);
   const float target = u * total;
   const float excl = base + incl - loc;
@@ -2381,9 +2422,9 @@
   return tok;
 }
 
-__device__ __forceinline__ int sample_ll(const LLWord* ll, uint32_t ep, const LaunchParams& p, int pidx, const SampleArgs& a, unsigned char* scratch) {
-  if (a.top_p >= 1.0f && a.V <= 8 * kConsumerThreads && (a.V & 3) == 0) return sample_fast(ll, ep, &p, pidx, a, scratch);
-  return sample_row(nullptr, ll, ep, &p, pidx, a, sample_scratch(scratch));
+__device__ __forceinline__ int sample_ll(const LLWord* ll, uint32_t ep, const LaunchParams& p, int pidx, const SampleArgs* a, unsigned char* scratch) {
+  if (a->top_p >= 1.0f && a->V <= 8 * kConsumerThreads && (a->V & 3) == 0) return sample_fast(ll, ep, &p, pidx, a, scratch);
+  return sample_row(nullptr, ll, ep, &p, pidx, *a, sample_scratch(scratch));
 }
 
 __device__ __forceinline__ void publish_row(LLWord* dst, const bf16* src, int n, uint32_t ep) {
@@ -2401,22 +2442,46 @@
 __device__ __forceinline__ void sample_phase(const Phase& ph, const LaunchParams& p, unsigned char* smem_base, uint32_t ep, int pidx,
                              const int* frame_done) {
   const Smem sm = carve_smem(smem_base, p);
-  const SampleScratch sc = sample_scratch(sm.scratch);
   const int Ht = p.stacks[ST_TALKER].hidden;
   const int ncb = p.n_code_groups - 1;
   const uint32_t ep_in = ep - 1;
-  if ((int)blockIdx.x >= (p.mode == MODE_PREFILL ? 1 : p.n_rows) && threadIdx.x == 0 && ph.skind != SMP_PRED && ph.skind != SMP_PRED_ONLY)
+  SampleArgs* const a = reinterpret_cast<SampleArgs*>(smem_base + kSampleArgsOffset);
+  SampleCtx* const cx = reinterpret_cast<SampleCtx*>(smem_base + kSampleCtxOffset);
+  const bool pred = ph.skind == SMP_PRED || ph.skind == SMP_PRED_ONLY;
+  if ((int)blockIdx.x >= (p.mode == MODE_PREFILL ? 1 : p.n_rows) && threadIdx.x == 0 && !pred)
     __threadfence();
   for (int b = blockIdx.x; b < (p.mode == MODE_PREFILL ? 1 : p.n_rows); b += gridDim.x) {
     prof_mark(p, pidx, 0);
-    cbar_sync();
     const int slot = p.stream0 + b;
     StreamState* st = p.st + slot;
+    if (threadIdx.x == 0) {
+      if (pred) {
+        const int Vp = p.stacks[ST_PRED].vocab;
+        a->V = Vp; a->do_sample = p.sub.do_sample; a->top_k = p.sub.top_k; a->top_p = p.sub.top_p;
+        a->temperature = p.sub.temperature; a->rep_pen = 1.0f; a->seen = nullptr; a->seen8 = nullptr; a->suppress_start = Vp;
+        a->eos = -1; a->suppress_eos = 0; a->round_bf16 = 1; a->seed = cx->key;
+        a->draw = cx->draws + (unsigned long long)(ph.aux + 1);
+        a->next_emb = p.pred_embeds[ph.aux]; a->emb_row_bytes = Ht * 2;
+      } else {
+        const int Vt = p.stacks[ST_TALKER].vocab;
+        const int nfr = cx->n_frames;
+        const Policy& pol = cx->pol;
+        const bool pen = ph.skind == SMP_TALKER && nfr > 0;
+        a->V = Vt; a->do_sample = pol.do_sample; a->top_k = pol.top_k; a->top_p = pol.top_p;
+        a->temperature = pol.temperature; a->rep_pen = pol.rep_pen;
+        a->seen = pen ? st->seen : nullptr; a->seen8 = pen ? cx->seen8 : nullptr;
+        a->suppress_start = max(0, Vt - pol.suppress_tail); a->eos = p.eos_id;
+        a->suppress_eos = (ph.skind == SMP_PREFILL) ? (pol.min_new_tokens > 0) : (nfr < pol.min_new_tokens);
+        a->round_bf16 = 1; a->seed = cx->key; a->draw = cx->draws;
+        a->next_emb = p.codec_embed; a->emb_row_bytes = Ht * 2;
+      }
+    }
+    cbar_sync();
     const int done = (p.mode == MODE_FRAMES) ? frame_done[b] : 0;
     LLWord* pin = reinterpret_cast<LLWord*>(p.bufs[p.has_s2m ? BUF_PIN : BUF_PX]);
     const int ldpin = p.ld[p.has_s2m ? BUF_PIN : BUF_PX];
     const LLWord* lgbuf = reinterpret_cast<const LLWord*>(p.bufs[BUF_LOGITS]);
-    if (ph.skind == SMP_PRED || ph.skind == SMP_PRED_ONLY) {
+    if (pred) {
       const int i = ph.aux;
       const int Vp = p.stacks[ST_PRED].vocab;
       const int lrow = (ph.flags & F_ROWS2) ? 2 * b + 1 : b;
@@ -2428,94 +2493,70 @@
           p.pred_logits_all[(size_t)i * Vp + 2 * v + 1] = bf_hi(pay);
         }
       }
-      const bool own = p.spol != nullptr && __ldcg(&p.spol[slot].on) != 0;
-      const unsigned long long seed = own ? __ldcg(&p.spol[slot].pol.seed) : p.pol.seed;
-      SampleArgs a;
-      a.V = Vp; a.do_sample = p.sub.do_sample; a.top_k = p.sub.top_k; a.top_p = p.sub.top_p;
-      a.temperature = p.sub.temperature; a.rep_pen = 1.0f; a.seen = nullptr; a.suppress_start = Vp; a.eos = -1;
-      a.suppress_eos = 0; a.round_bf16 = 1; a.seed = seed ^ (0x9E3779B97F4A7C15ull * (unsigned long long)(own ? 1 : slot + 1));
-      a.draw = __ldcg(&st->draws) + (unsigned long long)(i + 1);
-      a.next_emb = p.pred_embeds[i]; a.emb_row_bytes = Ht * 2;
       const int tok = sample_ll(lg, ep_in, p, pidx, a, sm.scratch);
       FQ3_ASSERT(tok >= 0 && tok < Vp, pidx, 100000 + tok);
-      if (threadIdx.x == 0) st->cur_codes[i + 1] = tok;
+      if (threadIdx.x == 0) { st->cur_codes[i + 1] = tok; cx->cur_codes[i + 1] = tok; }
       if (i + 1 < ncb) {
         publish_row(pin + (size_t)b * ldpin, p.pred_embeds[i] + (size_t)tok * Ht, Ht, ep);
       } else if (ph.skind == SMP_PRED) {
-        const int nfr = __ldcg(&st->n_frames);
-        const int c0 = __ldcg(&st->token);
-        if (!done) {
-          if (threadIdx.x < p.n_code_groups && nfr < p.max_frames) {
-            const int code = (threadIdx.x == 0) ? c0 : (threadIdx.x == ncb ? tok : __ldcg(&st->cur_codes[threadIdx.x]));
-            st->codes[(size_t)nfr * p.n_code_groups + threadIdx.x] = code;
-          }
-          if (threadIdx.x == 0) {
-            st->n_frames = nfr + 1;
-            st->seen[c0] = 1;
-            st->draws = __ldcg(&st->draws) + 32ull;
-          }
-        }
-        cbar_sync();
-        const int gs = __ldcg(&st->gen_step);
-        const int ntr = __ldcg(&st->n_trailing);
+        const int nfr = cx->n_frames;
+        const int c0 = cx->token;
+        if (!done && threadIdx.x < p.n_code_groups && nfr < p.max_frames) {
+          const int code = (threadIdx.x == 0) ? c0 : (threadIdx.x == ncb ? tok : cx->cur_codes[threadIdx.x]);
+          st->codes[(size_t)nfr * p.n_code_groups + threadIdx.x] = code;
+        }
+        const int gs = cx->gen_step;
+        const int ntr = cx->n_trailing;
         const bf16* text = (gs < ntr) ? st->trailing + (size_t)gs * Ht : st->pad_embed;
         LLWord* tx = reinterpret_cast<LLWord*>(p.bufs[BUF_TX]) + (size_t)b * p.ld[BUF_TX];
         const uint32_t* ce = reinterpret_cast<const uint32_t*>(p.codec_embed + (size_t)c0 * Ht);
         const uint32_t* tx32 = reinterpret_cast<const uint32_t*>(text);
         for (int c = threadIdx.x; c < (Ht >> 1); c += kConsumerThreads) {
-          uint32_t v = __ldg(ce + c);
+          const uint32_t v = __ldg(ce + c);
+          const uint32_t t = __ldg(tx32 + c);
           float s0 = bf_lo(v), s1 = bf_hi(v);
-          for (int g = 0; g < ncb; ++g) {
-            const int code = (g == ncb - 1) ? tok : __ldcg(&st->cur_codes[g + 1]);
-            v = __ldg(reinterpret_cast<const uint32_t*>(p.pred_embeds[g] + (size_t)code * Ht) + c);
-            s0 += bf_lo(v); s1 += bf_hi(v);
+          for (int g0 = 0; g0 < ncb; g0 += 8) {
+            uint32_t w[8];
+#pragma unroll
+            for (int r = 0; r < 8; ++r) {
+              const int g = min(g0 + r, ncb - 1);
+              const int code = (g == ncb - 1) ? tok : cx->cur_codes[g + 1];
+              w[r] = __ldg(reinterpret_cast<const uint32_t*>(p.pred_embeds[g] + (size_t)code * Ht) + c);
+            }
+#pragma unroll
+            for (int r = 0; r < 8; ++r)
+              if (g0 + r < ncb) { s0 += bf_lo(w[r]); s1 += bf_hi(w[r]); }
           }
-          const uint32_t t = __ldg(tx32 + c);
           ll_st(tx + c, pack_bf16x2(bf16r(bf16r(s0) + bf_lo(t)), bf16r(bf16r(s1) + bf_hi(t))), ep);
         }
+        cbar_sync();
         if (threadIdx.x == 0 && !done) {
-          const int pos = __ldcg(&st->position);
-          if (pos >= p.stacks[ST_TALKER].max_pos - 1) st->done = 2;
+          st->n_frames = nfr + 1; cx->n_frames = nfr + 1;
+          st->seen[c0] = 1; cx->seen8[c0 >> 3] |= (uint8_t)(1u << (c0 & 7));
+          st->draws = cx->draws + 32ull; cx->draws += 32ull;
+          if (cx->position >= p.stacks[ST_TALKER].max_pos - 1) { st->done = 2; cx->done = 2; }
         }
       }
     } else {
-      const int Vt = p.stacks[ST_TALKER].vocab;
       const LLWord* lg = lgbuf + (size_t)b * p.ld[BUF_LOGITS];
-      const int nfr = __ldcg(&st->n_frames);
-      const int done_now = (ph.skind == SMP_PREFILL) ? 0 : __ldcg(&st->done);
-      const bool own = p.spol != nullptr && __ldcg(&p.spol[slot].on) != 0;
-      Policy pol;
-      if (own) {
-        const Policy* sp = &p.spol[slot].pol;
-        pol.do_sample = __ldcg(&sp->do_sample); pol.top_k = __ldcg(&sp->top_k); pol.top_p = __ldcg(&sp->top_p);
-        pol.temperature = __ldcg(&sp->temperature); pol.rep_pen = __ldcg(&sp->rep_pen);
-        pol.min_new_tokens = __ldcg(&sp->min_new_tokens); pol.suppress_tail = __ldcg(&sp->suppress_tail); pol.seed = __ldcg(&sp->seed);
-      } else {
-        pol = p.pol;
-      }
-      SampleArgs a;
-      a.V = Vt; a.do_sample = pol.do_sample; a.top_k = pol.top_k; a.top_p = pol.top_p;
-      a.temperature = pol.temperature; a.rep_pen = pol.rep_pen;
-      a.seen = (ph.skind == SMP_TALKER && nfr > 0) ? st->seen : nullptr;
-      a.suppress_start = max(0, Vt - pol.suppress_tail); a.eos = p.eos_id;
-      a.suppress_eos = (ph.skind == SMP_PREFILL) ? (pol.min_new_tokens > 0) : (nfr < pol.min_new_tokens);
-      a.round_bf16 = 1;
-      a.seed = pol.seed ^ (0x9E3779B97F4A7C15ull * (unsigned long long)(own ? 1 : slot + 1));
-      a.draw = __ldcg(&st->draws);
-      a.next_emb = p.codec_embed; a.emb_row_bytes = Ht * 2;
       int tok = sample_ll(lg, ep_in, p, pidx, a, sm.scratch);
+      const int done_now = (ph.skind == SMP_PREFILL) ? 0 : cx->done;
       const bool live = !done_now;
-      int new_done = done_now, new_pos = __ldcg(&st->position), new_gs = __ldcg(&st->gen_step);
+      int new_done = done_now, new_pos = cx->position, new_gs = cx->gen_step;
       if (live) {
         if (ph.skind == SMP_TALKER) { new_pos += 1; new_gs += 1; }
         if (tok == p.eos_id) new_done = 1;
-        else if (__ldcg(&st->text_open) && new_gs >= __ldcg(&st->n_trailing)) new_done = 4;
+        else if (cx->text_open && new_gs >= cx->n_trailing) new_done = 4;
       } else {
-        tok = __ldcg(&st->token);
+        tok = cx->token;
       }
       cbar_sync();
       if (threadIdx.x == 0) {
-        if (live) { st->token = tok; st->draws = a.draw + 1ull; st->position = new_pos; st->gen_step = new_gs; st->done = new_done; }
+        if (live) {
+          const unsigned long long dr = cx->draws + 1ull;
+          st->token = tok; st->draws = dr; st->position = new_pos; st->gen_step = new_gs; st->done = new_done;
+          cx->token = tok; cx->draws = dr; cx->position = new_pos; cx->gen_step = new_gs; cx->done = new_done;
+        }
         ll_st(&st->ctl[0], (uint32_t)new_done, ep);
         ll_st(&st->ctl[1], (uint32_t)new_pos, ep);
       }
@@ -2615,6 +2656,9 @@
   uint32_t gst = 0u;
   int* frame_pos = sm.ctl + kFramePosIdx;
   int* frame_done = sm.ctl + kFrameDoneIdx;
+  if ((p.mode == MODE_FRAMES || p.mode == MODE_PREDICTOR || p.mode == MODE_PREFILL) &&
+      (int)blockIdx.x < (p.mode == MODE_PREFILL ? 1 : p.n_rows))
+    load_sample_ctx(p, reinterpret_cast<SampleCtx*>(smem_raw + kSampleCtxOffset));
   for (int iter = 0; iter < p.n_iters; ++iter) {
     const uint32_t ep0 = p.epoch_base + (uint32_t)iter * (uint32_t)p.n_phases;
     if (p.mode == MODE_FRAMES || p.mode == MODE_TALKER_STEP) {
```

New measurement: 46.74 (median of 6 runs). No clear change (+0.9%).
